# hustvl/ControlAR

Hardware: AMD Instinct MI355X
Metric: images/sec/GPU, LlamaGen-XL t2i canny 512x512 (1024 tok); 1/2/4/8-GPU scaling (higher is better)
Workload: dtype bf16

## Files before the change

controlar_amd/csrc/decode2.hip:

```cpp
#include "car_common.h"

typedef __attribute__((ext_vector_type(4))) unsigned u32x4;
typedef __attribute__((ext_vector_type(2))) float f32x2_t;
typedef __attribute__((ext_vector_type(2))) __bf16 bf16x2_t;

__device__ inline unsigned pack_bf16x2(float a, float b) {
    const f32x2_t v = {a, b};
    const bf16x2_t r = __builtin_convertvector(v, bf16x2_t);
    return *(const unsigned*)&r;
}

#include "decode2_params.h"

#ifdef CAR_STAMP
#define STAMP(p, i) do { if (threadIdx.x == 0 && (p).stamp) { const int wg_ = (int)(blockIdx.x + gridDim.x * (blockIdx.y + gridDim.y * blockIdx.z)); \
    if (wg_ < 2048) (p).stamp[((long)(p).stamp_slot * 2048 + wg_) * 8 + (i)] = (long long)wall_clock64(); } } while (0)
#else
#define STAMP(p, i) do { } while (0)
#endif

template <typename P>
__device__ inline void car_pf_helper_kv(const P& p, int hidx, unsigned& acc) {
    if (!p.pf_kc) return;
    const int x = (int)(blockIdx.x & 7), R = p.pf_wgs >> 3, r = hidx >> 3, nth = (int)blockDim.x, tid = (int)threadIdx.x;
    if (r >= R) return;
    const int pos = *p.pf_pos;
    const unsigned L = (unsigned)((((pos >> 5) + 1) * 32 * 64 * p.pf_kvb) >> 7);
    const unsigned nix = (unsigned)((p.pf_items - x + 7) >> 3);
    const unsigned tot = nix * 2u * L, step = (unsigned)(R * nth);
    const size_t stream = (size_t)p.pf_SA * 64 * p.pf_kvb;
    for (unsigned i = (unsigned)(r * nth + tid); i < tot; i += step) {
        const unsigned it = i / (2u * L), rem = i - it * 2u * L;
        const char* base = (const char*)(rem < L ? p.pf_kc : p.pf_vc) + (size_t)(x + 8 * (int)it) * stream;
        acc ^= *(const unsigned*)(base + (size_t)(rem < L ? rem : rem - L) * 128);
    }
}
__device__ inline void car_pf_helper(const void* p0, unsigned b0, const void* p1, unsigned b1, int hidx, int pf_wgs) {
    const int x = (int)(blockIdx.x & 7), R = pf_wgs >> 3, r = hidx >> 3, nth = (int)blockDim.x, tid = (int)threadIdx.x;
    if (r >= R) return;
    unsigned acc = 0;
#pragma unroll
    for (int job = 0; job < 2; ++job) {
        const unsigned* q = (const unsigned*)(job ? p1 : p0);
        const unsigned lines = (job ? b1 : b0) >> 7;
        if (!q || !lines) continue;
        const unsigned per = (lines + 7) >> 3, lo = (unsigned)x * per, hi = lo + per < lines ? lo + per : lines;
        const unsigned step = (unsigned)(R * nth);
        for (unsigned i = lo + (unsigned)(r * nth + tid); i < hi; i += step * 8) {
            unsigned v[8];
#pragma unroll
            for (int u = 0; u < 8; ++u) { const unsigned j = i + (unsigned)u * step; v[u] = 0; if (j < hi) v[u] = q[(size_t)j * 32]; }
#pragma unroll
            for (int u = 0; u < 8; ++u) acc ^= v[u];
        }
    }
    asm volatile("" ::"v"(acc));
}

typedef __attribute__((address_space(1))) const void car_gptr_t;
typedef __attribute__((address_space(3))) void car_lptr_t;

__device__ inline float sat448(float v) { return __builtin_amdgcn_fmed3f(v, -448.0f, 448.0f); }

__device__ inline bf16x8 fp8x8_to_bf16x8_(unsigned lo, unsigned hi) {
    const bf16x2_t a = __builtin_amdgcn_cvt_scalef32_pk_bf16_fp8(lo, 1.0f, false), b = __builtin_amdgcn_cvt_scalef32_pk_bf16_fp8(lo, 1.0f, true);
    const bf16x2_t c = __builtin_amdgcn_cvt_scalef32_pk_bf16_fp8(hi, 1.0f, false), d = __builtin_amdgcn_cvt_scalef32_pk_bf16_fp8(hi, 1.0f, true);
    u32x4 r;
    r[0] = *(const unsigned*)&a; r[1] = *(const unsigned*)&b; r[2] = *(const unsigned*)&c; r[3] = *(const unsigned*)&d;
    return *(bf16x8*)&r;
}

__device__ inline long bf16x8_to_fp8x8_(const u32x4 x) {
    int lo = 0, hi = 0;
#define CL(v) __builtin_amdgcn_fmed3f((v), -448.0f, 448.0f)
    lo = __builtin_amdgcn_cvt_pk_fp8_f32(CL(__uint_as_float(x[0] << 16)), CL(__uint_as_float(x[0] & 0xffff0000u)), lo, false);
    lo = __builtin_amdgcn_cvt_pk_fp8_f32(CL(__uint_as_float(x[1] << 16)), CL(__uint_as_float(x[1] & 0xffff0000u)), lo, true);
    hi = __builtin_amdgcn_cvt_pk_fp8_f32(CL(__uint_as_float(x[2] << 16)), CL(__uint_as_float(x[2] & 0xffff0000u)), hi, false);
    hi = __builtin_amdgcn_cvt_pk_fp8_f32(CL(__uint_as_float(x[3] << 16)), CL(__uint_as_float(x[3] & 0xffff0000u)), hi, true);
#undef CL
    return (long)(((unsigned long long)(unsigned)hi << 32) | (unsigned long long)(unsigned)lo);
}

template <int I, int J, int WAVES, int EPI, int F8, int NORM>
__global__ __launch_bounds__(WAVES * 64) void dec_gemm_kernel(GemmDP p) {
    extern __shared__ __attribute__((aligned(16))) float red_all[];
    static_assert((NORM != 1 && NORM != 3) || J == 1, "the prologue-norm and staged-norm variants serve one m-block");
    const int xs_ld = p.K + 8;
    bf16_t* xs = (bf16_t*)red_all;
    float* red = NORM == 1 ? red_all + (16 * xs_ld) / 2 : (NORM == 3 ? red_all + ((size_t)WAVES * p.stg) / 4 : red_all);
    constexpr int XPU = F8 ? 2 : 1;
    if (J == 1 && WAVES >= 8) car_kernarg_prefetch<(sizeof(GemmDP) + 63 + 48) / 64>();
    const int tid = threadIdx.x, lane = tid & 63, wave = tid >> 6;
    if (p.pf_wgs > 0 && (int)blockIdx.x >= (int)gridDim.x - p.pf_wgs) {
        STAMP(p, 0);
        car_pf_helper(p.pf_p0, p.pf_b0, p.pf_p1, p.pf_b1, (int)blockIdx.x - ((int)gridDim.x - p.pf_wgs), p.pf_wgs);
        { unsigned acc = 0; car_pf_helper_kv(p, (int)blockIdx.x - ((int)gridDim.x - p.pf_wgs), acc); asm volatile("" ::"v"(acc)); }
        STAMP(p, 5);
        return;
    }
    if (p.w_nt & 2) __builtin_amdgcn_s_setprio(3);
    STAMP(p, 0);
    const int nkb = p.K >> 5, nku = nkb / XPU, Mb = (p.M + 15) >> 4;
    const int MT = (Mb + J - 1) / J;
    int t = blockIdx.x; const int total = (int)gridDim.x - p.pf_wgs;
    if ((total & 7) == 0) t = (t & 7) * (total >> 3) + (t >> 3);
    const int nt = (NORM == 3) ? t : t / MT, mt = t - nt * MT;
    const int rb0 = nt * I, mb0 = mt * J;
    const int jn = (Mb - mb0) < J ? (Mb - mb0) : J;
    const int ku_lo = (int)((long)nku * wave / WAVES), ku_hi = (int)((long)nku * (wave + 1) / WAVES);
    const u32x4* wp = (const u32x4*)p.W + (long)rb0 * nku * 64 + lane;
    const u32x4* xp = (const u32x4*)p.X + (long)mb0 * nkb * 64 + lane;

    f32x4 acc[I][J];
#pragma unroll
    for (int i = 0; i < I; ++i)
#pragma unroll
        for (int j = 0; j < J; ++j) acc[i][j] = (f32x4){0.f, 0.f, 0.f, 0.f};
    const u32x4 zw = (u32x4){0u, 0u, 0u, 0u};
    constexpr int DEPTH = WAVES == 16 ? 8 : ((28 / (I + J * XPU)) < 2 ? 2 : ((28 / (I + J * XPU)) > 6 ? 6 : (28 / (I + J * XPU))));
    u32x4 wr[DEPTH][I], xr[DEPTH][J * XPU], nr[DEPTH][NORM == 2 ? XPU : 1];
    const bf16_t* hrow[J]; bool hok[J]; float rstd[J];
#pragma unroll
    for (int j = 0; j < J; ++j) { const int m = (mb0 + j) * 16 + (lane & 15); hok[j] = NORM == 2 && m < p.M; hrow[j] = NORM == 2 ? p.nh_in + (long)(hok[j] ? m : 0) * p.K + (lane >> 4) * 8 : nullptr; rstd[j] = 0.f; }
    auto loadW = [&](u32x4 (&w)[I], u32x4 (&nwf)[NORM == 2 ? XPU : 1], int ku) {
#pragma unroll
        for (int i = 0; i < I; ++i) {
            const u32x4* a = wp + ((long)i * nku + ku) * 64;
            w[i] = (p.w_nt & 1) ? __builtin_nontemporal_load(a) : *a;
        }
        if (NORM == 2) {
#pragma unroll
            for (int u = 0; u < XPU; ++u) nwf[u] = *(const u32x4*)(p.nw + (ku * XPU + u) * 32 + (lane >> 4) * 8);
        }
    };
    auto loadX = [&](u32x4 (&x)[J * XPU], int ku) {
        if (NORM == 0) {
#pragma unroll
            for (int j = 0; j < J; ++j)
#pragma unroll
                for (int u = 0; u < XPU; ++u) { x[j * XPU + u] = zw; if (j < jn) x[j * XPU + u] = xp[((long)j * nkb + ku * XPU + u) * 64]; }
        } else if (NORM == 2) {
#pragma unroll
            for (int j = 0; j < J; ++j)
#pragma unroll
                for (int u = 0; u < XPU; ++u) { x[j * XPU + u] = zw; if (hok[j]) x[j * XPU + u] = *(const u32x4*)(hrow[j] + (ku * XPU + u) * 32); }
        }
    };
    auto load = [&](u32x4 (&w)[I], u32x4 (&x)[J * XPU], u32x4 (&nwf)[NORM == 2 ? XPU : 1], int ku) { loadW(w, nwf, ku); loadX(x, ku); };
    const bf16_t* xl = xs + (lane & 15) * xs_ld + (lane >> 4) * 8;
    const int s_nkbw = NORM == 3 ? (ku_hi - ku_lo) * XPU : 0;
    const int s_xr = NORM == 3 ? (p.M * ((nku + WAVES - 1) / WAVES) * XPU * 4 + 63) >> 6 : 0;
    const int s_row = (lane & 15) < p.M ? (lane & 15) : p.M - 1;
    const char* stg_x = (const char*)red_all + (size_t)wave * (NORM == 3 ? p.stg : 0);
    const char* stg_w = stg_x + (size_t)s_xr * 1024;
    const char* stg_s = stg_w + 1024;
    auto compute = [&](const u32x4 (&w)[I], u32x4 (&x)[J * XPU], const u32x4 (&nwf)[NORM == 2 ? XPU : 1], int ku) {
        if (NORM == 1) {
#pragma unroll
            for (int u = 0; u < XPU; ++u) x[u] = *(const u32x4*)(xl + (ku * XPU + u) * 32);
        } else if (NORM == 3) {
#pragma unroll
            for (int u = 0; u < XPU; ++u) {
                const int kq = ((ku - ku_lo) * XPU + u) * 4 + (lane >> 4);
                x[u] = *(const u32x4*)(stg_x + ((size_t)s_row * (s_nkbw * 4) + kq) * 16);
                const u32x4 wq = *(const u32x4*)(stg_w + (size_t)kq * 16);
#pragma unroll
                for (int e = 0; e < 4; ++e) {
                    const unsigned hv = x[u][e], wv = wq[e];
                    const unsigned t = pack_bf16x2(__uint_as_float(hv << 16) * rstd[0], __uint_as_float(hv & 0xffff0000u) * rstd[0]);
                    x[u][e] = pack_bf16x2(__uint_as_float(t << 16) * __uint_as_float(wv << 16), __uint_as_float(t & 0xffff0000u) * __uint_as_float(wv & 0xffff0000u));
                }
            }
        } else if (NORM == 2) {
#pragma unroll
            for (int j = 0; j < J; ++j)
#pragma unroll
                for (int u = 0; u < XPU; ++u)
#pragma unroll
                    for (int e = 0; e < 4; ++e) {
                        const unsigned hv = x[j * XPU + u][e], wv = nwf[u][e];
                        const unsigned t = pack_bf16x2(__uint_as_float(hv << 16) * rstd[j], __uint_as_float(hv & 0xffff0000u) * rstd[j]);
                        x[j * XPU + u][e] = pack_bf16x2(__uint_as_float(t << 16) * __uint_as_float(wv << 16), __uint_as_float(t & 0xffff0000u) * __uint_as_float(wv & 0xffff0000u));
                    }
        }
        long x8[J][2];
        if (F8 == 2) {
#pragma unroll
            for (int j = 0; j < J; ++j) { x8[j][0] = bf16x8_to_fp8x8_(x[j * XPU]); x8[j][1] = bf16x8_to_fp8x8_(x[j * XPU + XPU - 1]); }
        }
#pragma unroll
        for (int i = 0; i < I; ++i) {
            if (F8 == 2) {
                const long a0 = (long)(((unsigned long long)w[i][1] << 32) | w[i][0]), a1 = (long)(((unsigned long long)w[i][3] << 32) | w[i][2]);
#pragma unroll
                for (int j = 0; j < J; ++j) {
                    acc[i][j] = __builtin_amdgcn_mfma_f32_16x16x32_fp8_fp8(a0, x8[j][0], acc[i][j], 0, 0, 0);
                    acc[i][j] = __builtin_amdgcn_mfma_f32_16x16x32_fp8_fp8(a1, x8[j][1], acc[i][j], 0, 0, 0);
                }
            } else if (F8) {
                const bf16x8 a0 = fp8x8_to_bf16x8_(w[i][0], w[i][1]), a1 = fp8x8_to_bf16x8_(w[i][2], w[i][3]);
#pragma unroll
                for (int j = 0; j < J; ++j) {
                    acc[i][j] = __builtin_amdgcn_mfma_f32_16x16x32_bf16(a0, *(const bf16x8*)&x[j * XPU], acc[i][j], 0, 0, 0);
                    acc[i][j] = __builtin_amdgcn_mfma_f32_16x16x32_bf16(a1, *(const bf16x8*)&x[j * XPU + XPU - 1], acc[i][j], 0, 0, 0);
                }
            } else {
#pragma unroll
                for (int j = 0; j < J; ++j)
                    acc[i][j] = __builtin_amdgcn_mfma_f32_16x16x32_bf16(*(const bf16x8*)&w[i], *(const bf16x8*)&x[j], acc[i][j], 0, 0, 0);
            }
        }
    };
    const int nkw = ku_hi - ku_lo;
    uint2 nh[8], na[8], nwv[8];
    bool n_add = false;
    if (NORM == 1) {
        const int D = p.K, ng = D >> 2;
        if (wave < p.M) {
            const int m = wave;
            const bf16_t* src = p.nidx ? p.nemb + (long)p.nidx[m] * D : p.nh_in + (long)m * D;
            const bf16_t* add = p.nadd ? p.nctrl + ((long)m * p.n_tok + (*p.pos - p.nT + 1)) * D : nullptr;
            n_add = add != nullptr;
#pragma unroll
            for (int q = 0; q < 8; ++q) {
                const int gi = lane + q * 64;
                if (gi < ng) { nh[q] = *(const uint2*)(src + gi * 4); nwv[q] = *(const uint2*)(p.nw + gi * 4); if (add) na[q] = *(const uint2*)(add + gi * 4); }
            }
        }
    }
    float4 sv[(NORM == 2 && J <= 2) ? J : 1][8];
    auto ssq_issue = [&](float4 (&v)[8], int j) {
        const int np4 = p.ssq_np >> 2, q4n = lane >> 4;
        const float4* sp = (const float4*)(p.ssq_in + (long)((mb0 + j) * 16 + (lane & 15)) * p.ssq_np);
#pragma unroll
        for (int t = 0; t < 8; ++t) { v[t] = make_float4(0.f, 0.f, 0.f, 0.f); if (hok[j] && q4n + 4 * t < np4) { const u32x4 r = *(const u32x4*)(sp + q4n + 4 * t); v[t] = make_float4(__uint_as_float(r[0]), __uint_as_float(r[1]), __uint_as_float(r[2]), __uint_as_float(r[3])); } }
    };
    auto ssq_finish = [&](const float4 (&v)[8], int j) {
        float sum = 0.f;
#pragma unroll
        for (int t = 0; t < 8; ++t) { sum += v[t].x; sum += v[t].y; sum += v[t].z; sum += v[t].w; }
        sum += __shfl_xor(sum, 16, 64); sum += __shfl_xor(sum, 32, 64);
        rstd[j] = hok[j] ? rsqrtf(sum / p.K + p.neps) : 0.f;
    };
    constexpr int IPc = I >= 2 ? I / 2 : 1, IWc = I >= 2 ? 2 : 1;
    const bool epi_first = wave < IPc * J && p.M <= 16;
    uint2 hv_h[IWc]; float4 cs_h[IWc];
    int pos_h = 0;
    if (EPI == EPI_QKV && p.M <= 16) pos_h = *(const __attribute__((address_space(4))) int*)(unsigned long long)p.pos;
    if (EPI == EPI_RESID && epi_first) {
        const int ip0 = wave / J, j0 = wave - ip0 * J;
        int m0 = (mb0 + j0) * 16 + (lane & 15); m0 = m0 < p.M ? m0 : p.M - 1;
#pragma unroll
        for (int ii = 0; ii < IWc; ++ii) hv_h[ii] = *(const uint2*)(p.h + (long)m0 * p.N + (rb0 + ip0 * IWc + ii) * 16 + (lane >> 4) * 4);
    }
    auto rope_first = [&]() {
        if (EPI == EPI_QKV && epi_first) {
            const int ip0 = wave / J;
#pragma unroll
            for (int ii = 0; ii < IWc; ++ii) {
                const int n0 = (rb0 + ip0 * IWc + ii) * 16 + (lane >> 4) * 4, d0 = (n0 % p.dim) & 63;
                cs_h[ii] = *(const float4*)(p.rope + ((long)pos_h * 32 + (d0 >> 1)) * 2);
            }
        }
    };
    if (NORM == 3 && s_nkbw > 0) {
        const int c4 = s_nkbw * 4, xtot = p.M * c4, kb0 = ku_lo * XPU;
        for (int r = 0; r < s_xr; ++r) {
            int ci = lane + 64 * r; ci = ci < xtot ? ci : xtot - 1;
            const int m = ci / c4, k8 = ci - m * c4;
            __builtin_amdgcn_global_load_lds((car_gptr_t*)(p.nh_in + (long)m * p.K + kb0 * 32 + k8 * 8), (car_lptr_t*)(stg_x + (size_t)r * 1024), 16, 0, 0);
        }
        { const int ci = lane < c4 ? lane : c4 - 1;
          __builtin_amdgcn_global_load_lds((car_gptr_t*)(p.nw + kb0 * 32 + ci * 8), (car_lptr_t*)stg_w, 16, 0, 0); }
        const int stot = p.M * (p.ssq_np >> 2), sr = (stot + 63) >> 6;
        for (int r = 0; r < sr; ++r) {
            int ci = lane + 64 * r; ci = ci < stot ? ci : stot - 1;
            __builtin_amdgcn_global_load_lds((car_gptr_t*)(p.ssq_in + (long)ci * 4), (car_lptr_t*)(stg_s + (size_t)r * 1024), 16, 0, 0);
        }
    }
    if (NORM == 2) {
#pragma unroll
        for (int j = 0; j < J; ++j) { if (J <= 2) ssq_issue(sv[j], j); else { ssq_issue(sv[0], j); ssq_finish(sv[0], j); } }
    }
#pragma unroll
    for (int d = 0; d < DEPTH; ++d) if (d < nkw) load(wr[d], xr[d], nr[d], ku_lo + d);
    rope_first();
    STAMP(p, 6);
    if (NORM == 3) {
        asm volatile("s_waitcnt vmcnt(0)" ::: "memory");
        const int np4 = p.ssq_np >> 2, q4n = lane >> 4;
        float sum = 0.f;
        for (int t = 0; 4 * t < np4; ++t) {
            const int ci = q4n + 4 * t;
            const float4 v = *(const float4*)(stg_s + ((size_t)s_row * np4 + (ci < np4 ? ci : np4 - 1)) * 16);
            const bool ok = ci < np4;
            sum += ok ? v.x : 0.f; sum += ok ? v.y : 0.f; sum += ok ? v.z : 0.f; sum += ok ? v.w : 0.f;
        }
        sum += __shfl_xor(sum, 16, 64); sum += __shfl_xor(sum, 32, 64);
        rstd[0] = (lane & 15) < p.M ? rsqrtf(sum / p.K + p.neps) : 0.f;
    }
    if (NORM == 2 && J <= 2) {
#pragma unroll
        for (int j = 0; j < J; ++j) ssq_finish(sv[J <= 2 ? j : 0], j);
    }
    if (NORM == 1) {
        const int D = p.K, ng = D >> 2;
        for (int m = wave; m < p.M; m += WAVES) {
            if (m != wave) {
                const bf16_t* src = p.nidx ? p.nemb + (long)p.nidx[m] * D : p.nh_in + (long)m * D;
                const bf16_t* add = p.nadd ? p.nctrl + ((long)m * p.n_tok + (*p.pos - p.nT + 1)) * D : nullptr;
                n_add = add != nullptr;
#pragma unroll
                for (int q = 0; q < 8; ++q) {
                    const int gi = lane + q * 64;
                    if (gi < ng) { nh[q] = *(const uint2*)(src + gi * 4); if (add) na[q] = *(const uint2*)(add + gi * 4); }
                }
            }
            float val[8][4];
            float ss = 0.f;
#pragma unroll
            for (int q = 0; q < 8; ++q) {
                const int gi = lane + q * 64;
                if (gi < ng) {
                    const uint2 u = nh[q];
                    float v[4] = {__uint_as_float(u.x << 16), __uint_as_float(u.x & 0xffff0000u), __uint_as_float(u.y << 16), __uint_as_float(u.y & 0xffff0000u)};
                    if (n_add) {
                        const uint2 a = na[q];
                        const float c[4] = {__uint_as_float(a.x << 16), __uint_as_float(a.x & 0xffff0000u), __uint_as_float(a.y << 16), __uint_as_float(a.y & 0xffff0000u)};
#pragma unroll
                        for (int e = 0; e < 4; ++e) v[e] = bf2f(f2bf(v[e] + bf2f(f2bf(p.ncs * c[e]))));
                    }
#pragma unroll
                    for (int e = 0; e < 4; ++e) { val[q][e] = v[e]; ss += v[e] * v[e]; }
                }
            }
            const float rstd = rsqrtf(wave_sum(ss) / D + p.neps);
#pragma unroll
            for (int q = 0; q < 8; ++q) {
                const int gi = lane + q * 64;
                if (gi < ng) {
                    const int k = gi * 4;
                    if (p.nh_out && blockIdx.x == 0) { uint2 u; u.x = pack_bf16x2(val[q][0], val[q][1]); u.y = pack_bf16x2(val[q][2], val[q][3]); *(uint2*)(p.nh_out + (long)m * D + k) = u; }
                    const uint2 wu = nwv[q];
                    const float w[4] = {__uint_as_float(wu.x << 16), __uint_as_float(wu.x & 0xffff0000u), __uint_as_float(wu.y << 16), __uint_as_float(wu.y & 0xffff0000u)};
                    uint2 u;
                    u.x = pack_bf16x2(bf2f(f2bf(val[q][0] * rstd)) * w[0], bf2f(f2bf(val[q][1] * rstd)) * w[1]);
                    u.y = pack_bf16x2(bf2f(f2bf(val[q][2] * rstd)) * w[2], bf2f(f2bf(val[q][3] * rstd)) * w[3]);
                    *(uint2*)(xs + m * xs_ld + k) = u;
                }
            }
        }
        __syncthreads();
    }
    STAMP(p, 1);
    for (int base = 0; base < nkw; base += DEPTH) {
#pragma unroll
        for (int d = 0; d < DEPTH; ++d) {
            if (base + d < nkw) {
                compute(wr[d], xr[d], nr[d], ku_lo + base + d);
#ifdef CAR_STAMP
                if (base + d == 0) { asm volatile("s_nop 0" ::"v"(acc[0][0][0])); STAMP(p, 2); }
#endif
                if (base + d + DEPTH < nkw) load(wr[d], xr[d], nr[d], ku_lo + base + d + DEPTH);
            }
        }
    }
    f32x4* rv = (f32x4*)red;
#ifdef CAR_STAMP
    asm volatile("s_nop 0" ::"v"(acc[0][0][0])); STAMP(p, 3);
#endif
#pragma unroll
    for (int i = 0; i < I; ++i)
#pragma unroll
        for (int j = 0; j < J; ++j) rv[((wave * I + i) * J + j) * 64 + lane] = acc[i][j];
    __syncthreads();
    STAMP(p, 4);
    auto fold = [&](int i, int j) -> f32x4 {
        f32x4 s = rv[((0 * I + i) * J + j) * 64 + lane];
        for (int w = 1; w < WAVES; ++w) { const f32x4 v = rv[((w * I + i) * J + j) * 64 + lane]; s[0] += v[0]; s[1] += v[1]; s[2] += v[2]; s[3] += v[3]; }
        return s;
    };
    constexpr int IP = I >= 2 ? I / 2 : 1, IW = I >= 2 ? 2 : 1;
    const int q4 = lane >> 4, c16 = lane & 15;
    for (int u = wave; u < IP * J; u += WAVES) {
        const bool first_u = u == wave && epi_first;
        const int ip = u / J, j = u - ip * J;
        if (j >= jn) continue;
        const int m = (mb0 + j) * 16 + c16;
        f32x4 v[IW];
#pragma unroll
        for (int ii = 0; ii < IW; ++ii) {
            v[ii] = fold(ip * IW + ii, j);
            if (F8) {
                const float4 sc = *(const float4*)(p.wscale + (rb0 + ip * IW + ii) * 16 + q4 * 4);
                v[ii][0] *= sc.x; v[ii][1] *= sc.y; v[ii][2] *= sc.z; v[ii][3] *= sc.w;
            }
        }
        if (m >= p.M) continue;
        if (EPI == EPI_SWIGLU) {
            float s[4];
#pragma unroll
            for (int r = 0; r < 4; ++r) {
                const float a = bf2f(f2bf(v[0][r])), g = bf2f(f2bf(v[IW - 1][r]));
                s[r] = bf2f(f2bf(silu_f(a))) * g;
            }
            const int hid = ((rb0 >> 1) + ip) * 16 + q4 * 4;
            const int nkb2 = p.N >> 6;
            const long off = ((((long)(m >> 4) * nkb2 + (hid >> 5)) * 64 + ((hid & 31) >> 3) * 16 + (m & 15)) << 3) + (hid & 7);
            uint2 o; o.x = pack_bf16x2(s[0], s[1]); o.y = pack_bf16x2(s[2], s[3]);
            *(uint2*)(p.outp + off) = o;
        } else {
            float ssq_acc = 0.f;
#pragma unroll
            for (int ii = 0; ii < IW; ++ii) {
                const int n0 = (rb0 + ip * IW + ii) * 16 + q4 * 4;
                const f32x4 a = v[ii];
                if (EPI == EPI_LOGITS) {
                    float4 o; o.x = bf2f(f2bf(a[0])); o.y = bf2f(f2bf(a[1])); o.z = bf2f(f2bf(a[2])); o.w = bf2f(f2bf(a[3]));
                    *(float4*)(p.outf + (long)m * p.N + n0) = o;
                } else if (EPI == EPI_RESID) {
                    bf16_t* hp = p.h + (long)m * p.N + n0;
                    const uint2 hv = first_u ? hv_h[ii] : *(const uint2*)hp;
                    const float h0 = __uint_as_float(hv.x << 16), h1 = __uint_as_float(hv.x & 0xffff0000u);
                    const float h2 = __uint_as_float(hv.y << 16), h3 = __uint_as_float(hv.y & 0xffff0000u);
                    uint2 o;
                    o.x = pack_bf16x2(h0 + bf2f(f2bf(a[0])), h1 + bf2f(f2bf(a[1])));
                    o.y = pack_bf16x2(h2 + bf2f(f2bf(a[2])), h3 + bf2f(f2bf(a[3])));
                    *(uint2*)hp = o;
                    if (p.ssq_out) {
                        const float s0 = __uint_as_float(o.x << 16), s1 = __uint_as_float(o.x & 0xffff0000u), s2 = __uint_as_float(o.y << 16), s3 = __uint_as_float(o.y & 0xffff0000u);
                        ssq_acc += s0 * s0; ssq_acc += s1 * s1; ssq_acc += s2 * s2; ssq_acc += s3 * s3;
                    }
                } else {
                    const int pos = p.M <= 16 ? pos_h : *p.pos;
                    const int sec = n0 / p.dim, within = n0 - sec * p.dim, hh = within >> 6, d0 = within & 63;
                    const float x0 = bf2f(f2bf(a[0])), x1 = bf2f(f2bf(a[1])), x2 = bf2f(f2bf(a[2])), x3 = bf2f(f2bf(a[3]));
                    const long sb = ((long)m * p.H + hh) * p.SA * 64;
                    if (sec == 2) {
                        const int w = pos & 31, qv = w < 16 ? (w >> 2) : ((w - 16) >> 2), ev = w < 16 ? (w & 3) : (4 + ((w - 16) & 3));
                        if (p.kv8) {
                            unsigned char* vb = (unsigned char*)p.vc + sb + (long)(pos >> 5) * 2048 + (d0 >> 5) * 1024 + ((qv * 16 + (d0 & 15)) << 4) + ((d0 >> 4) & 1) * 8 + ev;
                            const int e01 = __builtin_amdgcn_cvt_pk_fp8_f32(sat448(x0), sat448(x1), 0, false), e23 = __builtin_amdgcn_cvt_pk_fp8_f32(sat448(x2), sat448(x3), 0, false);
                            vb[0] = (unsigned char)(e01 & 0xff); vb[16] = (unsigned char)((e01 >> 8) & 0xff); vb[32] = (unsigned char)(e23 & 0xff); vb[48] = (unsigned char)((e23 >> 8) & 0xff);
                        } else {
                            bf16_t* vb = p.vc + sb + ((long)(pos >> 5) * 4 + (d0 >> 4)) * 512 + ((qv * 16 + (d0 & 15)) << 3) + ev;
                            vb[0] = f2bf(x0); vb[8] = f2bf(x1); vb[16] = f2bf(x2); vb[24] = f2bf(x3);
                        }
                    } else {
                        const float4 cs = first_u ? cs_h[ii] : *(const float4*)(p.rope + ((long)pos * 32 + (d0 >> 1)) * 2);
                        const float r0 = x0 * cs.x - x1 * cs.y, r1 = x1 * cs.x + x0 * cs.y;
                        const float r2 = x2 * cs.z - x3 * cs.w, r3 = x3 * cs.z + x2 * cs.w;
                        if (sec == 0) {
                            uint2 o;
                            o.x = pack_bf16x2(bf2f(f2bf(r0)) * 0.125f, bf2f(f2bf(r1)) * 0.125f);
                            o.y = pack_bf16x2(bf2f(f2bf(r2)) * 0.125f, bf2f(f2bf(r3)) * 0.125f);
                            *(uint2*)(p.qout + ((long)m * p.H + hh) * 64 + d0) = o;
                        } else if (p.kv8) {
                            unsigned char* kb_ = (unsigned char*)p.kc + sb + (long)(pos >> 4) * 1024 + ((((d0 & 31) >> 3) * 16 + (pos & 15)) << 4) + (d0 >> 5) * 8 + (d0 & 7);
                            int e = __builtin_amdgcn_cvt_pk_fp8_f32(sat448(bf2f(f2bf(r0))), sat448(bf2f(f2bf(r1))), 0, false);
                            e = __builtin_amdgcn_cvt_pk_fp8_f32(sat448(bf2f(f2bf(r2))), sat448(bf2f(f2bf(r3))), e, true);
                            *(unsigned*)kb_ = (unsigned)e;
                        } else {
                            uint2 o; o.x = pack_bf16x2(r0, r1); o.y = pack_bf16x2(r2, r3);
                            bf16_t* kb_ = p.kc + sb + ((long)(pos >> 4) * 2 + (d0 >> 5)) * 512 + ((((d0 & 31) >> 3) * 16 + (pos & 15)) << 3) + (d0 & 7);
                            *(uint2*)kb_ = o;
                        }
                    }
                }
            }
            if (EPI == EPI_RESID && p.ssq_out) {
                ssq_acc += __shfl_xor(ssq_acc, 16, 64); ssq_acc += __shfl_xor(ssq_acc, 32, 64);
                if (q4 == 0) *(unsigned*)(p.ssq_out + (long)m * p.ssq_ld + (rb0 / IW + ip)) = __float_as_uint(ssq_acc);
            }
        }
    }
#ifdef CAR_STAMP
    __builtin_amdgcn_s_waitcnt(0); STAMP(p, 5);
#endif
}

template <int I, int J, int WAVES, int F8, int NORM>
static void launch_gemm_ij(const GemmDP& p_, int epi, hipStream_t st) {
    GemmDP p = p_;
    const int Mb = (p.M + 15) / 16, MT = (Mb + J - 1) / J, NT = p.N / (16 * I);
    const dim3 g(NT * MT + (p.pf_wgs > 0 ? p.pf_wgs : 0)), b(WAVES * 64);
    if (NORM == 3) {
        const int nku = p.K / (F8 ? 64 : 32), xr = (p.M * ((nku + WAVES - 1) / WAVES) * (F8 ? 2 : 1) * 4 + 63) / 64, sr = (p.M * (p.ssq_np / 4) + 63) / 64;
        p.stg = (xr + 1 + sr) * 1024;
    }
    const size_t sh = (size_t)WAVES * I * J * 64 * 16 + (NORM == 1 ? (size_t)16 * (p.K + 8) * 2 : 0) + (NORM == 3 ? (size_t)WAVES * p.stg : 0);
    static size_t attr[4] = {0, 0, 0, 0};
#define LG(E)                                                                                                                   \
    do {                                                                                                                        \
        if (sh > 48 * 1024 && sh > attr[E]) { (void)hipFuncSetAttribute((const void*)dec_gemm_kernel<I, J, WAVES, E, F8, NORM>, hipFuncAttributeMaxDynamicSharedMemorySize, (int)sh); attr[E] = sh; } \
        hipLaunchKernelGGL((dec_gemm_kernel<I, J, WAVES, E, F8, NORM>), g, b, sh, st, p);                                        \
    } while (0)
    if (NORM) {
        if (epi == EPI_LOGITS) LG(EPI_LOGITS); else if (epi == EPI_SWIGLU) LG(EPI_SWIGLU); else LG(EPI_QKV);
    } else {
        if (epi == EPI_LOGITS) LG(EPI_LOGITS); else if (epi == EPI_RESID) LG(EPI_RESID); else if (epi == EPI_SWIGLU) LG(EPI_SWIGLU); else LG(EPI_QKV);
    }
#undef LG
}

extern "C" int car_launch_dec_gemm_cfg_ex(const GemmDP* p, int epi, int cfg, int staged_ok, hipStream_t st) {
    if (epi == EPI_SWIGLU && cfg < 200) return -1;
    if (p->N % (16 * (cfg / 100)) || p->K % 32) return -1;
    if (p->wscale && p->K % 64) return -1;
    const int f8 = p->wscale ? (p->f8_mfma ? 2 : 1) : 0;
    if (p->ssq_in) {
        if (!p->nw || !p->nh_in || epi == EPI_RESID || p->ssq_np <= 0 || (p->ssq_np & 3) || p->ssq_np > 128) return -1;
        {
            const int nku = p->K / (f8 ? 64 : 32), nkw_max = (nku + 7) / 8;
            if (p->M <= 16 && (cfg / 10) % 10 == 1 && cfg % 10 == 1 && nku >= 8 && nkw_max * (f8 ? 2 : 1) <= 16 && staged_ok) {
                switch (cfg / 100) {
#define CASE3(I) case I: if (f8 == 2) launch_gemm_ij<I, 1, 8, 2, 3>(*p, epi, st); else if (f8) launch_gemm_ij<I, 1, 8, 1, 3>(*p, epi, st); else launch_gemm_ij<I, 1, 8, 0, 3>(*p, epi, st); return 0;
                    CASE3(1) CASE3(2) CASE3(4)
#undef CASE3
                    default: break;
                }
            }
        }
        switch (cfg) {
#define CASE(I, J) case I * 100 + J * 10: if (f8 == 2) launch_gemm_ij<I, J, 4, 2, 2>(*p, epi, st); else if (f8) launch_gemm_ij<I, J, 4, 1, 2>(*p, epi, st); else launch_gemm_ij<I, J, 4, 0, 2>(*p, epi, st); break; \
                   case I * 100 + J * 10 + 1: if (f8 == 2) launch_gemm_ij<I, J, 8, 2, 2>(*p, epi, st); else if (f8) launch_gemm_ij<I, J, 8, 1, 2>(*p, epi, st); else launch_gemm_ij<I, J, 8, 0, 2>(*p, epi, st); break;
            CASE(1, 1) CASE(1, 2) CASE(1, 4) CASE(2, 1) CASE(2, 2) CASE(2, 4) CASE(4, 1) CASE(4, 2) CASE(4, 4)
#undef CASE
            default: return -1;
        }
        return 0;
    }
    if (p->nw) {
        if (p->M > 16 || (cfg / 10) % 10 != 1 || epi == EPI_RESID || p->K > 2048) return -1;
        switch (cfg) {
#define CASE(I) case I * 100 + 10: if (f8 == 2) launch_gemm_ij<I, 1, 4, 2, 1>(*p, epi, st); else if (f8) launch_gemm_ij<I, 1, 4, 1, 1>(*p, epi, st); else launch_gemm_ij<I, 1, 4, 0, 1>(*p, epi, st); break; \
                case I * 100 + 11: if (f8 == 2) launch_gemm_ij<I, 1, 8, 2, 1>(*p, epi, st); else if (f8) launch_gemm_ij<I, 1, 8, 1, 1>(*p, epi, st); else launch_gemm_ij<I, 1, 8, 0, 1>(*p, epi, st); break;
            CASE(1) CASE(2) CASE(4)
#undef CASE
            default: return -1;
        }
        return 0;
    }
    switch (cfg) {
#define CASE(I, J) case I * 100 + J * 10: if (f8 == 2) launch_gemm_ij<I, J, 4, 2, 0>(*p, epi, st); else if (f8) launch_gemm_ij<I, J, 4, 1, 0>(*p, epi, st); else launch_gemm_ij<I, J, 4, 0, 0>(*p, epi, st); break; \
                   case I * 100 + J * 10 + 1: if (f8 == 2) launch_gemm_ij<I, J, 8, 2, 0>(*p, epi, st); else if (f8) launch_gemm_ij<I, J, 8, 1, 0>(*p, epi, st); else launch_gemm_ij<I, J, 8, 0, 0>(*p, epi, st); break;
        CASE(1, 1) CASE(1, 2) CASE(1, 4) CASE(2, 1) CASE(2, 2) CASE(2, 4) CASE(4, 1) CASE(4, 2) CASE(4, 4)
#undef CASE
        case 112: if (f8 == 2) launch_gemm_ij<1, 1, 16, 2, 0>(*p, epi, st); else if (f8) launch_gemm_ij<1, 1, 16, 1, 0>(*p, epi, st); else launch_gemm_ij<1, 1, 16, 0, 0>(*p, epi, st); break;
        default: return -1;
    }
    return 0;
}

extern "C" int car_launch_dec_gemm_cfg(const GemmDP* p, int epi, int cfg, hipStream_t st) { return car_launch_dec_gemm_cfg_ex(p, epi, cfg, 1, st); }
extern "C" int car_pick_gemm_cfg(int M, int N, int K, int epi) {
    const int Mb = (M + 15) / 16;
    const bool wideN = N >= 6144, hugeN = N >= 16384, longK = K >= 2048, smallNK = N <= 1536 && K <= 1536;
    int cfg;
    if (Mb >= 12) cfg = wideN ? 440 : 241;
    else if (Mb >= 6) cfg = hugeN ? 440 : (wideN ? 441 : (smallNK ? 110 : 221));
    else if (Mb >= 3) cfg = hugeN ? 441 : (wideN ? 241 : (longK ? 211 : 110));
    else if (Mb == 2) cfg = hugeN ? 421 : (wideN ? 221 : (longK ? 121 : 120));
    else cfg = hugeN ? 411 : (wideN ? 211 : 111);
    if (Mb == 1 && epi == EPI_RESID && cfg == 111 && N / 16 <= 128) cfg = 112;
    int I = cfg / 100;
    if (epi == EPI_SWIGLU && I < 2) I = 2;
    while (I > 1 && N % (16 * I)) I >>= 1;
    return I * 100 + cfg % 100;
}

extern "C" void car_launch_dec_gemm(const GemmDP* p, int epi, hipStream_t st) {
    (void)car_launch_dec_gemm_cfg(p, epi, car_pick_gemm_cfg(p->M, p->N, p->K, epi), st);
}

template <int NWAVE, int PF, int KV8>
__global__ __launch_bounds__(NWAVE * 64) void dec_attn2_kernel(Attn2P p) {
    __shared__ float red[NWAVE][66];
    const int split = blockIdx.z;
    const int tid = threadIdx.x, lane = tid & 63, wave = tid >> 6, q4 = lane >> 4, c16 = lane & 15;
    STAMP(p, 0);
    const int pos = *p.pos;
    const bool persist = p.n_seq > 0;
    const int n_items = persist ? p.n_seq * p.H : 1;
    for (int it = persist ? (int)blockIdx.x : 0; it < n_items; it += gridDim.x) {
    const int h = persist ? it % p.H : (int)blockIdx.x, b = persist ? it / p.H : (int)blockIdx.y;
    const long sbase = ((long)b * p.H + h) * p.SA * 64;
    const u32x4* Kp = KV8 ? (const u32x4*)((const unsigned char*)p.kc + sbase) + lane : (const u32x4*)(p.kc + sbase) + lane;
    const u32x4* Vp = KV8 ? (const u32x4*)((const unsigned char*)p.vc + sbase) + lane : (const u32x4*)(p.vc + sbase) + lane;
    const bf16_t* qp = p.q + ((long)b * p.H + h) * 64;
    const bf16x8 qf0 = *(const bf16x8*)(qp + q4 * 8), qf1 = *(const bf16x8*)(qp + 32 + q4 * 8);
    const unsigned char* mk = p.mask ? p.mask + (long)b * p.T : nullptr;
    int jmin = 0;
    if (mk) {
        if (p.jmin) jmin = p.jmin[b];
        else {
            int jm = p.T;
            for (int j = lane; j < p.T; j += 64) { const int v = mk[j]; if (v != 0 && j < jm) jm = j; }
#pragma unroll
            for (int o = 32; o > 0; o >>= 1) jm = min(jm, __shfl_xor(jm, o, 64));
            jmin = jm;
        }
    }
    const int nblk = (pos >> 5) + 1, NW = p.nsplit * NWAVE;
    float m_run = -INFINITY, l_run = 0.f;
    f32x4 o[4];
#pragma unroll
    for (int d = 0; d < 4; ++d) o[d] = (f32x4){0.f, 0.f, 0.f, 0.f};
    const f32x4 z4 = (f32x4){0.f, 0.f, 0.f, 0.f};

    auto load = [&](u32x4 (&kr)[4], u32x4 (&vr)[4], unsigned (&mb)[8], int blk) {
        if (mk != nullptr && blk * 32 < p.T) {
            const int jb = blk * 32 + q4 * 4;
#pragma unroll
            for (int e = 0; e < 8; ++e) mb[e] = mk[min(jb + (e < 4 ? e : 12 + e), p.T - 1)];
        }
#pragma unroll
        for (int i = 0; i < (KV8 ? 2 : 4); ++i) kr[i] = __builtin_nontemporal_load(Kp + ((long)blk * (KV8 ? 2 : 4) + i) * 64);
#pragma unroll
        for (int i = 0; i < (KV8 ? 2 : 4); ++i) vr[i] = __builtin_nontemporal_load(Vp + ((long)blk * (KV8 ? 2 : 4) + i) * 64);
    };
    auto compute = [&](const u32x4 (&kr_)[4], const u32x4 (&vr_)[4], const unsigned (&mb)[8], int blk) {
        u32x4 kr[4], vr[4];
        if (KV8) {
#pragma unroll
            for (int i = 0; i < 2; ++i) {
                const bf16x8 a = fp8x8_to_bf16x8_(kr_[i][0], kr_[i][1]), c2 = fp8x8_to_bf16x8_(kr_[i][2], kr_[i][3]);
                const bf16x8 v0 = fp8x8_to_bf16x8_(vr_[i][0], vr_[i][1]), v1 = fp8x8_to_bf16x8_(vr_[i][2], vr_[i][3]);
                kr[2 * i] = *(const u32x4*)&a; kr[2 * i + 1] = *(const u32x4*)&c2; vr[2 * i] = *(const u32x4*)&v0; vr[2 * i + 1] = *(const u32x4*)&v1;
            }
        } else {
#pragma unroll
            for (int i = 0; i < 4; ++i) { kr[i] = kr_[i]; vr[i] = vr_[i]; }
        }
        f32x4 s0 = __builtin_amdgcn_mfma_f32_16x16x32_bf16(*(const bf16x8*)&kr[0], qf0, z4, 0, 0, 0);
        s0 = __builtin_amdgcn_mfma_f32_16x16x32_bf16(*(const bf16x8*)&kr[1], qf1, s0, 0, 0, 0);
        f32x4 s1 = __builtin_amdgcn_mfma_f32_16x16x32_bf16(*(const bf16x8*)&kr[2], qf0, z4, 0, 0, 0);
        s1 = __builtin_amdgcn_mfma_f32_16x16x32_bf16(*(const bf16x8*)&kr[3], qf1, s1, 0, 0, 0);
        float sc[8] = {s0[0], s0[1], s0[2], s0[3], s1[0], s1[1], s1[2], s1[3]};
        const int jb = blk * 32 + q4 * 4;
        const bool use_mk = mk != nullptr && blk * 32 < p.T;
        if (use_mk || blk * 32 + 31 > pos) {
#pragma unroll
            for (int e = 0; e < 8; ++e) {
                const int j = jb + (e < 4 ? e : 12 + e);
                unsigned mv = 1u;
                if (use_mk) mv = mb[e];
                const bool ok = (j <= pos) & ((j >= p.T) | (mv != 0u));
                sc[e] = ok ? sc[e] : -INFINITY;
            }
        }
        float mx = fmaxf(fmaxf(fmaxf(sc[0], sc[1]), fmaxf(sc[2], sc[3])), fmaxf(fmaxf(sc[4], sc[5]), fmaxf(sc[6], sc[7])));
        mx = fmaxf(mx, __shfl_xor(mx, 16, 64)); mx = fmaxf(mx, __shfl_xor(mx, 32, 64));
        if (mx > -INFINITY) {
            const float mn = fmaxf(m_run, mx), alpha = __expf(m_run - mn);
            float pe[8], ps = 0.f;
#pragma unroll
            for (int e = 0; e < 8; ++e) { pe[e] = __expf(sc[e] - mn); ps += pe[e]; }
            l_run = l_run * alpha + ps; m_run = mn;
            u32x4 pu; pu[0] = pack_bf16x2(pe[0], pe[1]); pu[1] = pack_bf16x2(pe[2], pe[3]); pu[2] = pack_bf16x2(pe[4], pe[5]); pu[3] = pack_bf16x2(pe[6], pe[7]);
#pragma unroll
            for (int d = 0; d < 4; ++d) {
                o[d][0] *= alpha; o[d][1] *= alpha; o[d][2] *= alpha; o[d][3] *= alpha;
                o[d] = __builtin_amdgcn_mfma_f32_16x16x32_bf16(*(const bf16x8*)&pu, *(const bf16x8*)&vr[d], o[d], 0, 0, 0);
            }
        }
    };
    if (PF) {
        u32x4 ka[4], va[4], kb2[4], vb2[4]; unsigned ma[8], mb2[8];
        int blk = (jmin >> 5) + split * NWAVE + wave;
        if (blk < nblk) load(ka, va, ma, blk);
        while (blk < nblk) {
            int nb = blk + NW;
            if (nb < nblk) load(kb2, vb2, mb2, nb);
            compute(ka, va, ma, blk);
            blk = nb;
            if (blk >= nblk) break;
            nb = blk + NW;
            if (nb < nblk) load(ka, va, ma, nb);
            compute(kb2, vb2, mb2, blk);
            blk = nb;
        }
    } else {
        u32x4 ka[4], va[4]; unsigned ma[8];
        for (int blk = (jmin >> 5) + split * NWAVE + wave; blk < nblk; blk += NW) { load(ka, va, ma, blk); compute(ka, va, ma, blk); }
    }
#ifdef CAR_STAMP
    asm volatile("s_nop 0" ::"v"(l_run)); STAMP(p, 3);
#endif
    float lt = l_run + __shfl_xor(l_run, 16, 64); lt += __shfl_xor(lt, 32, 64);
    if (q4 == 0) {
#pragma unroll
        for (int d = 0; d < 4; ++d) red[wave][2 + d * 16 + c16] = o[d][0];
    }
    if (lane == 0) { red[wave][0] = m_run; red[wave][1] = lt; }
    __syncthreads();
    STAMP(p, 4);
    if (tid < 64) {
        float M = red[0][0];
#pragma unroll
        for (int w = 1; w < NWAVE; ++w) M = fmaxf(M, red[w][0]);
        float L = 0.f, O = 0.f;
#pragma unroll
        for (int w = 0; w < NWAVE; ++w) {
            const float mm = red[w][0];
            const float a = mm > -INFINITY ? __expf(mm - M) : 0.f;
            L += red[w][1] * a; O += red[w][2 + tid] * a;
        }
        if (p.nsplit == 1) {
            const int k = h * 64 + tid;
            long off;
            if (p.out_packed) off = ((((long)(b >> 4) * (p.dim >> 5) + (k >> 5)) * 64 + ((k & 31) >> 3) * 16 + (b & 15)) << 3) + (k & 7);
            else off = (long)b * p.dim + k;
            p.out[off] = f2bf(O / L);
        } else {
            float* pt = p.part + (((long)b * p.H + h) * p.nsplit + split) * 66;
            if (tid == 0) { pt[0] = M; pt[1] = L; }
            pt[2 + tid] = O;
        }
    }
    if (persist) __syncthreads();
    }
    if (persist && p.pf_wgs > 0 && (int)blockIdx.x >= n_items) car_pf_helper(p.pf_p0, p.pf_b0, p.pf_p1, p.pf_b1, (int)blockIdx.x - n_items, p.pf_wgs);
#ifdef CAR_STAMP
    __builtin_amdgcn_s_waitcnt(0); STAMP(p, 5);
#endif
}

template <int KV8>
__global__ __launch_bounds__(1024) void dec_attn2s_kernel(Attn2P p) {
    __shared__ float red[16][66];
    car_kernarg_prefetch<(sizeof(Attn2P) + 63 + 48) / 64>();
    const int tid = threadIdx.x, lane = tid & 63, wave = tid >> 6, q4 = lane >> 4, c16 = lane & 15;
    STAMP(p, 0);
    const int n_items = p.n_seq * p.H;
    if ((int)blockIdx.x >= n_items) {
        car_pf_helper(p.pf_p0, p.pf_b0, p.pf_p1, p.pf_b1, (int)blockIdx.x - n_items, p.pf_wgs);
#ifdef CAR_STAMP
        __builtin_amdgcn_s_waitcnt(0); STAMP(p, 5);
#endif
        return;
    }
    const int h = (int)blockIdx.x % p.H, b = (int)blockIdx.x / p.H;
    const int pos = *p.pos;
    const unsigned char* mk = p.mask ? p.mask + (long)b * p.T : nullptr;
    const int jmin = mk ? p.jmin[b] : 0;
    const long sbase = ((long)b * p.H + h) * p.SA * 64;
    const u32x4* Kp = KV8 ? (const u32x4*)((const unsigned char*)p.kc + sbase) + lane : (const u32x4*)(p.kc + sbase) + lane;
    const u32x4* Vp = KV8 ? (const u32x4*)((const unsigned char*)p.vc + sbase) + lane : (const u32x4*)(p.vc + sbase) + lane;
    const bf16_t* qp = p.q + ((long)b * p.H + h) * 64;
    bf16x8 qf0, qf1;
    const int nblk = (pos >> 5) + 1;
    float m_run = -INFINITY, l_run = 0.f;
    f32x4 o[4];
#pragma unroll
    for (int d = 0; d < 4; ++d) o[d] = (f32x4){0.f, 0.f, 0.f, 0.f};
    const f32x4 z4 = (f32x4){0.f, 0.f, 0.f, 0.f};
    constexpr int NL = KV8 ? 2 : 4;
    auto loadkv = [&](u32x4 (&kr)[4], u32x4 (&vr)[4], int blk) {
#pragma unroll
        for (int i = 0; i < NL; ++i) kr[i] = __builtin_nontemporal_load(Kp + ((long)blk * NL + i) * 64);
#pragma unroll
        for (int i = 0; i < NL; ++i) vr[i] = __builtin_nontemporal_load(Vp + ((long)blk * NL + i) * 64);
    };
    unsigned ma[8];
    auto compute = [&](const u32x4 (&kr_)[4], const u32x4 (&vr_)[4], int blk, bool use_mk) {
        u32x4 kr[4], vr[4];
        if (KV8) {
#pragma unroll
            for (int i = 0; i < 2; ++i) {
                const bf16x8 a = fp8x8_to_bf16x8_(kr_[i][0], kr_[i][1]), c2 = fp8x8_to_bf16x8_(kr_[i][2], kr_[i][3]);
                const bf16x8 v0 = fp8x8_to_bf16x8_(vr_[i][0], vr_[i][1]), v1 = fp8x8_to_bf16x8_(vr_[i][2], vr_[i][3]);
                kr[2 * i] = *(const u32x4*)&a; kr[2 * i + 1] = *(const u32x4*)&c2; vr[2 * i] = *(const u32x4*)&v0; vr[2 * i + 1] = *(const u32x4*)&v1;
            }
        } else {
#pragma unroll
            for (int i = 0; i < 4; ++i) { kr[i] = kr_[i]; vr[i] = vr_[i]; }
        }
        f32x4 s0 = __builtin_amdgcn_mfma_f32_16x16x32_bf16(*(const bf16x8*)&kr[0], qf0, z4, 0, 0, 0);
        s0 = __builtin_amdgcn_mfma_f32_16x16x32_bf16(*(const bf16x8*)&kr[1], qf1, s0, 0, 0, 0);
        f32x4 s1 = __builtin_amdgcn_mfma_f32_16x16x32_bf16(*(const bf16x8*)&kr[2], qf0, z4, 0, 0, 0);
        s1 = __builtin_amdgcn_mfma_f32_16x16x32_bf16(*(const bf16x8*)&kr[3], qf1, s1, 0, 0, 0);
        float sc[8] = {s0[0], s0[1], s0[2], s0[3], s1[0], s1[1], s1[2], s1[3]};
        const int jb = blk * 32 + q4 * 4;
        if (use_mk || blk * 32 + 31 > pos) {
#pragma unroll
            for (int e = 0; e < 8; ++e) {
                const int j = jb + (e < 4 ? e : 12 + e);
                unsigned mv = 1u;
                if (use_mk) mv = ma[e];
                const bool ok = (j <= pos) & ((j >= p.T) | (mv != 0u));
                sc[e] = ok ? sc[e] : -INFINITY;
            }
        }
        float mx = fmaxf(fmaxf(fmaxf(sc[0], sc[1]), fmaxf(sc[2], sc[3])), fmaxf(fmaxf(sc[4], sc[5]), fmaxf(sc[6], sc[7])));
        mx = fmaxf(mx, __shfl_xor(mx, 16, 64)); mx = fmaxf(mx, __shfl_xor(mx, 32, 64));
        if (mx > -INFINITY) {
            const float mn = fmaxf(m_run, mx), alpha = __expf(m_run - mn);
            float pe[8], ps = 0.f;
#pragma unroll
            for (int e = 0; e < 8; ++e) { pe[e] = __expf(sc[e] - mn); ps += pe[e]; }
            l_run = l_run * alpha + ps; m_run = mn;
            u32x4 pu; pu[0] = pack_bf16x2(pe[0], pe[1]); pu[1] = pack_bf16x2(pe[2], pe[3]); pu[2] = pack_bf16x2(pe[4], pe[5]); pu[3] = pack_bf16x2(pe[6], pe[7]);
#pragma unroll
            for (int d = 0; d < 4; ++d) {
                o[d][0] *= alpha; o[d][1] *= alpha; o[d][2] *= alpha; o[d][3] *= alpha;
                o[d] = __builtin_amdgcn_mfma_f32_16x16x32_bf16(*(const bf16x8*)&pu, *(const bf16x8*)&vr[d], o[d], 0, 0, 0);
            }
        }
    };
    {
        u32x4 ka[4], va[4], kb2[4], vb2[4];
        int cur = (jmin >> 5) + wave;
        const bool mk_a = mk != nullptr && cur * 32 < p.T && cur < nblk;
        if (mk_a) {
            const int jb = cur * 32 + q4 * 4;
#pragma unroll
            for (int e = 0; e < 8; ++e) ma[e] = mk[min(jb + (e < 4 ? e : 12 + e), p.T - 1)];
        }
        if (cur < nblk) loadkv(ka, va, cur);
        if (cur + 16 < nblk) loadkv(kb2, vb2, cur + 16);
        { const u32x4 q0 = *(const u32x4*)(qp + q4 * 8), q1 = *(const u32x4*)(qp + 32 + q4 * 8); qf0 = *(const bf16x8*)&q0; qf1 = *(const bf16x8*)&q1; }
        bool first = true;
        while (cur < nblk) {
            compute(ka, va, cur, first && mk_a);
            first = false;
            if (cur + 32 < nblk) loadkv(ka, va, cur + 32);
            if (cur + 16 < nblk) { compute(kb2, vb2, cur + 16, false); if (cur + 48 < nblk) loadkv(kb2, vb2, cur + 48); }
            cur += 32;
        }
    }
#ifdef CAR_STAMP
    asm volatile("s_nop 0" ::"v"(l_run)); STAMP(p, 3);
#endif
    float lt = l_run + __shfl_xor(l_run, 16, 64); lt += __shfl_xor(lt, 32, 64);
    if (q4 == 0) {
#pragma unroll
        for (int d = 0; d < 4; ++d) red[wave][2 + d * 16 + c16] = o[d][0];
    }
    if (lane == 0) { red[wave][0] = m_run; red[wave][1] = lt; }
    __syncthreads();
    STAMP(p, 4);
    if (tid < 64) {
        float M = red[0][0];
#pragma unroll
        for (int w = 1; w < 16; ++w) M = fmaxf(M, red[w][0]);
        float L = 0.f, O = 0.f;
#pragma unroll
        for (int w = 0; w < 16; ++w) {
            const float mm = red[w][0];
            const float a = mm > -INFINITY ? __expf(mm - M) : 0.f;
            L += red[w][1] * a; O += red[w][2 + tid] * a;
        }
        const int k = h * 64 + tid;
        long off;
        if (p.out_packed) off = ((((long)(b >> 4) * (p.dim >> 5) + (k >> 5)) * 64 + ((k & 31) >> 3) * 16 + (b & 15)) << 3) + (k & 7);
        else off = (long)b * p.dim + k;
        p.out[off] = f2bf(O / L);
    }
#ifdef CAR_STAMP
    __builtin_amdgcn_s_waitcnt(0); STAMP(p, 5);
#endif
}

__global__ void build_mask_kernel(const int64_t* emb_mask, const int* row_img, unsigned char* out, int b, int T) {
    const long i = (long)blockIdx.x * blockDim.x + threadIdx.x;
    if (i >= (long)b * T) return;
    const int r = (int)(i / T), t = (int)(i - (long)r * T);
    out[i] = emb_mask ? (unsigned char)(emb_mask[(long)row_img[r] * T + t] != 0) : (unsigned char)1;
}
extern "C" void car_launch_build_mask(const int64_t* emb_mask, const int* row_img, unsigned char* out, int b, int T, hipStream_t st) {
    const long n = (long)b * T;
    hipLaunchKernelGGL(build_mask_kernel, dim3((unsigned)((n + 255) / 256)), dim3(256), 0, st, emb_mask, row_img, out, b, T);
}

__global__ void mask_first_valid_kernel(const unsigned char* mask, int* jmin, int T) {
    const int b = blockIdx.x, lane = threadIdx.x;
    int jm = T;
    for (int j = lane; j < T; j += 64) { const int v = mask[(long)b * T + j]; if (v != 0 && j < jm) jm = j; }
#pragma unroll
    for (int o = 32; o > 0; o >>= 1) jm = min(jm, __shfl_xor(jm, o, 64));
    if (lane == 0) jmin[b] = jm;
}
extern "C" void car_launch_mask_first_valid(const unsigned char* mask, int* jmin, int b, int T, hipStream_t st) {
    hipLaunchKernelGGL(mask_first_valid_kernel, dim3(b), dim3(64), 0, st, mask, jmin, T);
}
__global__ __launch_bounds__(256) void min_int_kernel(const int* v, int n, int* out, int need, int* flag) {
    __shared__ int sm[4];
    int m = 0x7fffffff;
    for (int i = threadIdx.x; i < n; i += 256) m = min(m, v[i]);
#pragma unroll
    for (int o = 32; o > 0; o >>= 1) m = min(m, __shfl_xor(m, o, 64));
    if ((threadIdx.x & 63) == 0) sm[threadIdx.x >> 6] = m;
    __syncthreads();
    if (threadIdx.x == 0) { const int r = min(min(sm[0], sm[1]), min(sm[2], sm[3])); out[0] = r; if (flag && need >= 0 && r < need) *flag = 1; }
}
extern "C" void car_launch_min_int(const int* v, int n, int* out, int need, int* flag, hipStream_t st) { hipLaunchKernelGGL(min_int_kernel, dim3(1), dim3(256), 0, st, v, n, out, need, flag); }

__global__ __launch_bounds__(64) void dec_attn2_combine_kernel(const float* part, bf16_t* out, int H, int nsplit, int dim, int out_packed) {
    const int h = blockIdx.x, b = blockIdx.y, d = threadIdx.x;
    const float* pt = part + ((long)b * H + h) * nsplit * 66;
    float M = -INFINITY;
    for (int s = 0; s < nsplit; ++s) M = fmaxf(M, pt[s * 66]);
    float L = 0.f, O = 0.f;
    for (int s = 0; s < nsplit; ++s) {
        const float mm = pt[s * 66];
        if (mm > -INFINITY) { const float a = __expf(mm - M); L += pt[s * 66 + 1] * a; O += pt[s * 66 + 2 + d] * a; }
    }
    const int k = h * 64 + d;
    long off;
    if (out_packed) off = ((((long)(b >> 4) * (dim >> 5) + (k >> 5)) * 64 + ((k & 31) >> 3) * 16 + (b & 15)) << 3) + (k & 7);
    else off = (long)b * dim + k;
    out[off] = f2bf(O / L);
}

extern "C" void car_launch_dec_attn2_var(const Attn2P* p, int b, int variant, int lds_pad, hipStream_t st) {
    if (variant == 162 && p->nsplit == 1 && p->T <= 512 && (!p->mask || p->jmin)) {
        Attn2P q = *p; q.n_seq = b; q.pgrid = 0;
        if (q.pf_wgs < 0 || ((b * q.H) & 7)) q.pf_wgs = 0;
        const dim3 g(b * q.H + q.pf_wgs);
        if (q.kv8) hipLaunchKernelGGL((dec_attn2s_kernel<1>), g, dim3(1024), 0, st, q); else hipLaunchKernelGGL((dec_attn2s_kernel<0>), g, dim3(1024), 0, st, q);
        return;
    }
    if (variant == 162) variant = 160;
    const bool persist = p->n_seq > 0 && p->pgrid > 0 && p->nsplit == 1;
    Attn2P q = *p; if (!persist) { q.n_seq = 0; q.pgrid = 0; q.pf_wgs = 0; }
    p = &q;
    const dim3 g = persist ? dim3(q.pgrid, 1, 1) : dim3(p->H, b, p->nsplit);
    const size_t sh = (size_t)(lds_pad > 0 ? lds_pad : 0);
#define LA(NW, PF_) do { if (p->kv8) hipLaunchKernelGGL((dec_attn2_kernel<NW, PF_, 1>), g, dim3(NW * 64), sh, st, *p); else hipLaunchKernelGGL((dec_attn2_kernel<NW, PF_, 0>), g, dim3(NW * 64), sh, st, *p); } while (0)
    switch (variant) {
        case 20: LA(2, 0); break;
        case 21: LA(2, 1); break;
        case 40: LA(4, 0); break;
        case 80: LA(8, 0); break;
        case 81: LA(8, 1); break;
        case 160: LA(16, 0); break;
        case 161: LA(16, 1); break;
        default: LA(4, 1); break;
    }
#undef LA
    if (p->nsplit > 1 && p->out)
        hipLaunchKernelGGL(dec_attn2_combine_kernel, dim3(p->H, b), dim3(64), 0, st, p->part, p->out, p->H, p->nsplit, p->dim, p->out_packed);
}
extern "C" void car_launch_dec_attn2(const Attn2P* p, int b, hipStream_t st) { car_launch_dec_attn2_var(p, b, 40, 0, st); }
__global__ void prefill_rope_kv2_kernel(bf16_t* qkv, bf16_t* kcache, bf16_t* vcache, const float* rope, int b, int Tn, int H, int dim, int SA, int kv8, int t0) {
    const long total = (long)b * Tn * H * 32;
    long i = (long)blockIdx.x * blockDim.x + threadIdx.x;
    const long stride = (long)gridDim.x * blockDim.x;
    for (; i < total; i += stride) {
        const int pr = (int)(i % 32); const int h = (int)((i / 32) % H); const int tw = (int)((i / (32L * H)) % Tn); const long bb = i / (32L * H * Tn);
        bf16_t* row = qkv + (bb * Tn + tw) * 3 * dim;
        const int t = tw + t0;
        const float cs = rope[((long)t * 32 + pr) * 2], sn = rope[((long)t * 32 + pr) * 2 + 1];
        const float q0 = bf2f(row[h * 64 + 2 * pr]), q1 = bf2f(row[h * 64 + 2 * pr + 1]);
        const float k0 = bf2f(row[dim + h * 64 + 2 * pr]), k1 = bf2f(row[dim + h * 64 + 2 * pr + 1]);
        row[h * 64 + 2 * pr] = f2bf(q0 * cs - q1 * sn); row[h * 64 + 2 * pr + 1] = f2bf(q1 * cs + q0 * sn);
        const bf16_t kr0 = f2bf(k0 * cs - k1 * sn), kr1 = f2bf(k1 * cs + k0 * sn);
        row[dim + h * 64 + 2 * pr] = kr0; row[dim + h * 64 + 2 * pr + 1] = kr1;
        const long sb = (bb * H + h) * (long)SA * 64;
        const int d = 2 * pr;
        const int w = t & 31, qv = w < 16 ? (w >> 2) : ((w - 16) >> 2), ev = w < 16 ? (w & 3) : (4 + ((w - 16) & 3));
        if (kv8) {
            const int ek = __builtin_amdgcn_cvt_pk_fp8_f32(sat448(bf2f(kr0)), sat448(bf2f(kr1)), 0, false);
            unsigned char* kp = (unsigned char*)kcache + sb + (long)(t >> 4) * 1024 + ((((d & 31) >> 3) * 16 + (t & 15)) << 4) + (d >> 5) * 8 + (d & 7);
            kp[0] = (unsigned char)(ek & 0xff); kp[1] = (unsigned char)((ek >> 8) & 0xff);
            const int ev2 = __builtin_amdgcn_cvt_pk_fp8_f32(sat448(bf2f(row[2 * dim + h * 64 + d])), sat448(bf2f(row[2 * dim + h * 64 + d + 1])), 0, false);
            unsigned char* vp = (unsigned char*)vcache + sb + (long)(t >> 5) * 2048 + (d >> 5) * 1024 + ((qv * 16 + (d & 15)) << 4) + ((d >> 4) & 1) * 8 + ev;
            vp[0] = (unsigned char)(ev2 & 0xff); vp[16] = (unsigned char)((ev2 >> 8) & 0xff);
        } else {
            bf16_t* kp = kcache + sb + ((long)(t >> 4) * 2 + (d >> 5)) * 512 + ((((d & 31) >> 3) * 16 + (t & 15)) << 3) + (d & 7);
            kp[0] = kr0; kp[1] = kr1;
            bf16_t* vp = vcache + sb + ((long)(t >> 5) * 4 + (d >> 4)) * 512 + ((qv * 16 + (d & 15)) << 3) + ev;
            vp[0] = row[2 * dim + h * 64 + d]; vp[8] = row[2 * dim + h * 64 + d + 1];
        }
    }
}
extern "C" void car_launch_prefill_rope_kv2(void* qkv, void* kc, void* vc, const float* rope, int b, int Tn, int H, int dim, int SA, int kv8, int t0, hipStream_t st) {
    long total = (long)b * Tn * H * 32; int g = (int)((total + 255) / 256); if (g > 4096) g = 4096;
    hipLaunchKernelGGL(prefill_rope_kv2_kernel, dim3(g), dim3(256), 0, st, (bf16_t*)qkv, (bf16_t*)kc, (bf16_t*)vc, rope, b, Tn, H, dim, SA, kv8, t0);
}

template <int NQ>
__global__ __launch_bounds__(256) void rmsnorm2_kernel(Norm2P p, int rows) {
    car_kernarg_prefetch<(sizeof(Norm2P) + 63 + 48) / 64>();
    if (p.pf_wgs > 0 && (int)blockIdx.x >= (int)gridDim.x - p.pf_wgs) {
        STAMP(p, 0);
        car_pf_helper(p.pf_p0, p.pf_b0, p.pf_p1, p.pf_b1, (int)blockIdx.x - ((int)gridDim.x - p.pf_wgs), p.pf_wgs);
        STAMP(p, 5);
        return;
    }
    const long r = (long)blockIdx.x * 4 + (threadIdx.x >> 6);
    STAMP(p, 0);
    if (r < rows) {
    const int lane = threadIdx.x & 63;
    const int D = p.D, ng = D >> 2;
    const bf16_t* src = p.idx ? p.emb + (long)p.idx[r] * D : p.h_in + r * D;
    if (p.add & 2) __builtin_amdgcn_s_setprio(3);
    const bf16_t* add = (p.add & 1) ? p.ctrl + (r * p.n_tok + (*p.pos - p.T + 1)) * D : nullptr;
    float val[NQ][4];
    float ss = 0.f;
    uint2 wreg[NQ];
#pragma unroll
    for (int q = 0; q < NQ; ++q) { const int gi = lane + q * 64; if (gi < ng) wreg[q] = *(const uint2*)(p.w + gi * 4); }
#pragma unroll
    for (int q = 0; q < NQ; ++q) {
        const int gi = lane + q * 64;
        if (gi < ng) {
            const uint2 u = *(const uint2*)(src + gi * 4);
            float v[4] = {__uint_as_float(u.x << 16), __uint_as_float(u.x & 0xffff0000u), __uint_as_float(u.y << 16), __uint_as_float(u.y & 0xffff0000u)};
            if (add) {
                const uint2 a = *(const uint2*)(add + gi * 4);
                const float c[4] = {__uint_as_float(a.x << 16), __uint_as_float(a.x & 0xffff0000u), __uint_as_float(a.y << 16), __uint_as_float(a.y & 0xffff0000u)};
#pragma unroll
                for (int e = 0; e < 4; ++e) v[e] = bf2f(f2bf(v[e] + bf2f(f2bf(p.cs * c[e]))));
            }
#pragma unroll
            for (int e = 0; e < 4; ++e) { val[q][e] = v[e]; ss += v[e] * v[e]; }
        }
    }
    const float rstd = rsqrtf(wave_sum(ss) / D + p.eps);
#ifdef CAR_STAMP
    asm volatile("s_nop 0" ::"v"(rstd)); STAMP(p, 3);
#endif
    const int nkb = D >> 5;
#pragma unroll
    for (int q = 0; q < NQ; ++q) {
        const int gi = lane + q * 64;
        if (gi < ng) {
            const int k = gi * 4;
            if (p.h_out) { uint2 u; u.x = pack_bf16x2(val[q][0], val[q][1]); u.y = pack_bf16x2(val[q][2], val[q][3]); *(uint2*)(p.h_out + r * D + k) = u; }
            const uint2 wu = wreg[q];
            const float w[4] = {__uint_as_float(wu.x << 16), __uint_as_float(wu.x & 0xffff0000u), __uint_as_float(wu.y << 16), __uint_as_float(wu.y & 0xffff0000u)};
            float o[4];
#pragma unroll
            for (int e = 0; e < 4; ++e) o[e] = bf2f(f2bf(val[q][e] * rstd)) * w[e];
            uint2 u; u.x = pack_bf16x2(o[0], o[1]); u.y = pack_bf16x2(o[2], o[3]);
            const long off = ((((r >> 4) * nkb + (k >> 5)) * 64 + ((k & 31) >> 3) * 16 + (r & 15)) << 3) + (k & 7);
            *(uint2*)(p.xn + off) = u;
        }
    }
    }
#ifdef CAR_STAMP
    __builtin_amdgcn_s_waitcnt(0); STAMP(p, 5);
#endif
}
extern "C" void car_launch_rmsnorm2(const Norm2P* p, long rows, hipStream_t st) {
    const int nq = (p->D / 4 + 63) / 64;
    Norm2P q = *p;
    const unsigned main_wgs = (unsigned)((rows + 3) / 4);
    if (q.pf_wgs < 0 || (main_wgs & 7)) q.pf_wgs = 0;
    const dim3 g(main_wgs + (unsigned)q.pf_wgs), b(256);
    if (nq <= 4) hipLaunchKernelGGL((rmsnorm2_kernel<4>), g, b, 0, st, q, (int)rows);
    else if (nq <= 8) hipLaunchKernelGGL((rmsnorm2_kernel<8>), g, b, 0, st, q, (int)rows);
    else hipLaunchKernelGGL((rmsnorm2_kernel<16>), g, b, 0, st, q, (int)rows);
}
```

controlar_amd/csrc/decode2_params.h:

```cpp
#pragma once
#include "car_common.h"

#define CAR_GEMMDP_DEFINED
#ifdef CAR_STAMP
#define CAR_STAMP_FIELDS long long* stamp; int stamp_slot;
#else
#define CAR_STAMP_FIELDS
#endif
enum { EPI_LOGITS = 0, EPI_RESID = 1, EPI_SWIGLU = 2, EPI_QKV = 3 };

#define CAR_PF_FIELDS const void* pf_p0; const void* pf_p1; unsigned pf_b0, pf_b1; int pf_wgs; const void* pf_kc; const void* pf_vc; const int* pf_pos; int pf_items, pf_SA, pf_kvb;

struct GemmDP {
    const bf16_t* W;
    const bf16_t* X;
    int M, N, K;
    int w_nt;
    int f8_mfma;
    const float* wscale;
    bf16_t* h;
    bf16_t* outp;
    float* outf;
    bf16_t* qout;
    bf16_t* kc; bf16_t* vc;
    const float* rope;
    const int* pos;
    int H, SA, dim;
    int kv8;
    const bf16_t* nh_in; const bf16_t* nemb; const int* nidx; bf16_t* nh_out; const bf16_t* nw; const bf16_t* nctrl;
    int nadd, nT, n_tok; float ncs, neps;
    const float* ssq_in; int ssq_np;
    int stg;
    float* ssq_out; int ssq_ld;
    CAR_PF_FIELDS
    CAR_STAMP_FIELDS
};

struct Attn2P {
    const bf16_t* q;
    const bf16_t* kc; const bf16_t* vc;
    const int* pos;
    const unsigned char* mask;
    const int* jmin;
    bf16_t* out;
    float* part;
    int H, SA, T, dim, nsplit, out_packed;
    int kv8;
    int n_seq, pgrid;
    CAR_PF_FIELDS
    CAR_STAMP_FIELDS
};

struct Norm2P {
    const bf16_t* h_in; const bf16_t* emb; const int* idx; bf16_t* h_out; bf16_t* xn; const bf16_t* w;
    const bf16_t* ctrl; const int* pos; int add ; int T; int n_tok; float cs;
    int D; float eps;
    CAR_PF_FIELDS
    CAR_STAMP_FIELDS
};
```

controlar_amd/csrc/engine_generate.hip:

```cpp
#include "engine_internal.h"

enum { RA_NONE = 0, RA_SMALL, RA_NX, RA_MID, kEarlyChain = 8, kNoOverride = -0x7fffffff };
struct ChainPlan {
    int b0, bg, nsplit;
    int attn_variant, attn_lds_pad, attn_pgrid;
    int fuse_norm, normx, normx_max, normx_j4, staged_normx;
    int runahead, kv_runahead;
};
struct DecodePlan {
    int mode, NG, mult, img0[9];
    int phase, gsteps, lin_prio, no_graph;
    int n_early;
    int f32_resid_cfg, f32_qkv_tiled_from;
    ChainPlan ch[9];
};
static int attn_splits(int wg) { int n = 1; while (wg * n < 1024 && n < 16) n *= 2; return n; }

static void plan_decode(DecodePlan& pl, const car_config& g, int mode, int n_cu, int B, bool use_cfg, int S_max, int nsteps, int skip, bool has_mask) {
    memset(&pl, 0, sizeof(pl));
    const bool fast = mode == CAR_BF16;
    const int D = g.dim, Hn = g.n_head, Fh = g.ffn_hidden, V = g.vocab_size, T = g.cls_token_num;
    const int mult = use_cfg ? 2 : 1, b = mult * B;
    auto num = [](const char* v, int dflt) { return v ? atoi(v) : dflt; };
    const char *k_chains = CAR_KNOB("CAR_CHAINS"), *k_one_max = CAR_KNOB("CAR_ONE_LAUNCH_MAX"), *k_variant = CAR_KNOB("CAR_ATTN_VARIANT"), *k_phase = CAR_KNOB("CAR_PHASE_OFFSET"), *k_form = CAR_KNOB("CAR_ATTN_F32_FORM");
    const bool single_chain = CAR_KNOB("CAR_SINGLE_CHAIN"), no_early = CAR_KNOB("CAR_NO_EARLY_CHAIN"), split_small = CAR_KNOB("CAR_ATTN_SPLIT_SMALL"), old_small = CAR_KNOB("CAR_ATTN_OLD_SMALL");
    const bool no_runahead = CAR_KNOB("CAR_NO_RUNAHEAD"), no_small_fuse = CAR_KNOB("CAR_NO_SMALL_FUSE"), no_normx = CAR_KNOB("CAR_NO_NORMX"), kv_runahead = CAR_KNOB("CAR_KV_RUNAHEAD"), no_staged = CAR_KNOB("CAR_NO_STAGED_NORMX");
    const int k_nsplit = num(CAR_KNOB("CAR_ATTN_NSPLIT"), 0), k_persist = num(CAR_KNOB("CAR_ATTN_PERSIST"), 0), lds_pad = num(CAR_KNOB("CAR_ATTN_LDS_PAD"), 0);
    const int normx_max = num(CAR_KNOB("CAR_NORMX_MAX"), 48), normx_j4 = num(CAR_KNOB("CAR_NORMX_J4"), 0) != 0, k_gsteps = num(CAR_KNOB("CAR_GRAPH_STEPS"), 1);
    pl.mode = mode; pl.mult = mult; pl.lin_prio = num(CAR_KNOB("CAR_LINEAR_PRIO"), 0) != 0;
    pl.no_graph = CAR_KNOB("CAR_NO_GRAPH") != nullptr;
    pl.f32_resid_cfg = num(CAR_KNOB("CAR_F32_RESID_CFG"), kNoOverride); pl.f32_qkv_tiled_from = num(CAR_KNOB("CAR_F32_QKV_TILED_FROM"), kNoOverride);

    int NG = b >= 192 ? 2 : 1;
    if (!fast && b >= 288) NG = 3;
    if (k_chains) { const int v = atoi(k_chains); if (v >= 1 && v <= 8 && B / v >= 2) NG = v; }
    if (single_chain || NG > B) NG = 1;
    pl.NG = NG; for (int gi = 0; gi <= NG; ++gi) pl.img0[gi] = (int)((long)B * gi / NG);
    pl.phase = NG >= 2 && (k_phase ? atoi(k_phase) != 0 : !fast);
    pl.gsteps = fast && k_gsteps >= 1 && k_gsteps <= 64 ? k_gsteps : 1;
    const int nsplit_exact = (S_max + AF_SPLIT - 1) / AF_SPLIT;
    const bool fused = (long)Hn * b >= 2048 && nsplit_exact <= 8;
    auto plan_exact = [&](ChainPlan& cp) { cp.nsplit = nsplit_exact; cp.attn_variant = fused ? num(k_form, cp.bg < b ? 3 : 1) : 0; };
    for (int gi = 0; gi < NG; ++gi) {
        ChainPlan& cp = pl.ch[gi]; const int bg = mult * (pl.img0[gi + 1] - pl.img0[gi]);
        cp.b0 = mult * pl.img0[gi]; cp.bg = bg;
        if (!fast) { plan_exact(cp); continue; }
        const bool one_launch = (long)bg * Hn <= num(k_one_max, T <= 512 ? 480 : 240) && !split_small;
        cp.nsplit = one_launch ? 1 : attn_splits(bg * Hn);
        if (k_nsplit == 1 || k_nsplit == 2 || k_nsplit == 4 || k_nsplit == 8 || k_nsplit == 16) cp.nsplit = k_nsplit;
        cp.attn_variant = (one_launch && cp.nsplit == 1) ? ((T <= 512 && !old_small) ? 162 : 160) : ((cp.nsplit == 1 && bg < 128) ? 20 : 40);
        cp.attn_variant = num(k_variant, cp.attn_variant); cp.attn_lds_pad = lds_pad;
        if (k_persist > 0 && k_persist <= 16 && cp.nsplit == 1) { const long items = (long)bg * Hn, cap = (long)n_cu * k_persist;
            if (items > cap) { const long per = (items + cap - 1) / cap; cp.attn_pgrid = (int)((items + per - 1) / per); }
        }
        cp.fuse_norm = bg <= 8 && D <= 2048 && !no_small_fuse;
        cp.normx_max = normx_max; cp.normx_j4 = normx_j4; cp.staged_normx = !no_staged;
        cp.normx = bg <= normx_max && D % 128 == 0 && D <= 2048 && !no_normx;
        if (n_cu >= 128 && !no_runahead) cp.runahead = bg <= 16 ? RA_SMALL : (bg != b ? RA_NONE : (bg <= normx_max ? RA_NX : RA_MID));
        cp.kv_runahead = kv_runahead && cp.attn_variant == 162 && ((bg * Hn) & 7) == 0;
    }
    if (!fast && NG == 3 && mult == 1 && !k_chains && !no_early) {
        const double P = (double)g.n_layer * (4.0 * D * D + 3.0 * (double)D * Fh) + (double)V * D;
        const int rows_star = (int)(0.087 * P / (8.0 * D * g.n_layer));
        const int attended0 = has_mask ? 24 : T;
        pl.n_early = std::min(rows_star - attended0 - skip, nsteps); if (pl.n_early < 8) pl.n_early = 0;
        pl.ch[kEarlyChain].bg = b; plan_exact(pl.ch[kEarlyChain]);
    }
}

struct FastBufs { bf16_t *xn, *att, *mid, *q; float* logits; float* attn_part; float* ssq; };
struct ChainBind { int *pos, *step; FastBufs fb; SampleP sp; };
struct StepBufs {
    void *h, *xn, *qkv, *att, *mid; float* part; float* logits; int* cur;
    int b, SA, n_tok; bool use_ctrl; float cs; const unsigned char* maskb; const int* jmin;
    ChainBind ch[9];
};

static int enqueue_decode_step_fast(car_ctx* c, const StepBufs& sb, const DecodePlan& pl, int ci, hipStream_t st, hipEvent_t phase_ev, hipStream_t phase_dst) {
    const car_config& g = c->cfg;
    const ChainPlan& cp = pl.ch[ci]; const ChainBind& cb = sb.ch[ci]; const FastBufs& fb = cb.fb;
    const int D = g.dim, Hn = g.n_head, Fh = g.ffn_hidden, li = g.n_layer / 3, V = g.vocab_size, T = g.cls_token_num;
    const int b = cp.bg, b0 = cp.b0, nsplit = cp.nsplit, SA = sb.SA, n_tok = sb.n_tok, prio = pl.lin_prio;
    const size_t kv_layer = (size_t)sb.b * Hn * SA * 64, kv_off = (size_t)b0 * Hn * SA * 64;
    bf16_t* h = (bf16_t*)sb.h + (size_t)b0 * D;
    const bool f8 = g.decode_weight_fp8 != 0;
    int nk = 0, bad_cfg = 0;
    const bool ra_lin = cp.runahead == RA_SMALL || cp.runahead == RA_NX, ra_norm = cp.runahead == RA_NX || cp.runahead == RA_MID;
    auto wimg = [&](const std::string& wname, const void*& ptr, unsigned& bytes, size_t cap = (size_t)24 << 20) {
        auto it = c->w.find(wname + (f8 ? "#pk8" : "#pk"));
        if (it == c->w.end()) { ptr = nullptr; bytes = 0; return; }
        ptr = it->second.p; bytes = (unsigned)std::min(it->second.bytes, cap);
    };
    auto helpers_for = [&](bool on, int main_wgs) -> int {
        if (!on || (main_wgs & 7)) return 0;
        const int n = std::min(((c->n_cu - main_wgs) / 8) * 8, 192);
        return n >= 32 ? n : 0;
    };
    auto ctrl_at = [&](int l) { return sb.use_ctrl && l < g.n_layer && l % li == 0 && l / li < 3; };
    auto gemm = [&](const std::string& wname, const bf16_t* X, int N, int K, int epi, GemmDP gp_) -> int {
        GemmDP p = gp_;
        p.W = (const bf16_t*)Wp(c, wname + (f8 ? "#pk8" : "#pk")); p.X = X; p.M = b; p.N = N; p.K = K;
        p.wscale = f8 ? (const float*)Wp(c, wname + "#sc") : nullptr; p.f8_mfma = g.decode_weight_fp8 == 2;
        int cfg = car_pick_gemm_cfg(b, N, K, epi);
        if (p.ssq_in && b > 48 && b <= 64 && cp.normx_j4) cfg = ((epi == EPI_SWIGLU || N >= 6144) ? 200 : 100) + 40 + 1;
        const int I = cfg / 100, J = (cfg / 10) % 10, Mb = (b + 15) / 16;
        p.w_nt = ((Mb + J - 1) / J == 1 ? 1 : 0) | (prio ? 2 : 0);
        if (p.pf_wgs > 0) p.pf_wgs = std::min(helpers_for(ra_lin, (N / (16 * I)) * ((Mb + J - 1) / J)), 160);
        if (p.ssq_out) p.ssq_ld = N / (16 * (I >= 2 ? 2 : 1));
        if (car_launch_dec_gemm_cfg_ex(&p, epi, cfg, cp.staged_normx, st)) bad_cfg = cfg;
        ++nk;
        return p.ssq_out ? p.ssq_ld : 0;
    };
    GemmDP z; memset(&z, 0, sizeof(z));
    int ssq_np = 0;
    bf16_t* hc = h;
    bf16_t* halt = (bf16_t*)sb.xn + (size_t)b0 * D;
    auto norm_kernel = [&](const std::string& wname, int l, const std::string& pf0, const std::string& pf1, size_t cap0 = (size_t)24 << 20) {
        Norm2P np; memset(&np, 0, sizeof(np));
        np.h_in = h; np.xn = fb.xn; np.w = (const bf16_t*)Wp(c, wname); np.D = D; np.eps = g.norm_eps; np.add = prio ? 2 : 0;
        if (l == 0) { np.emb = (const bf16_t*)Wp(c, "tok_embeddings.weight"); np.idx = sb.cur + b0; np.h_out = h; }
        if (l >= 0 && ctrl_at(l)) {
            np.add |= 1; np.ctrl = (const bf16_t*)c->ctrl[l / li].p + (size_t)b0 * n_tok * D; np.pos = cb.pos; np.T = T; np.n_tok = n_tok; np.cs = sb.cs; np.h_out = h;
        }
        np.pf_wgs = helpers_for(ra_norm, (b + 3) / 4);
        if (np.pf_wgs > 0) { wimg(pf0, np.pf_p0, np.pf_b0, cap0); if (!pf1.empty()) wimg(pf1, np.pf_p1, np.pf_b1); }
        car_launch_rmsnorm2(&np, b, st); ++nk;
    };
    auto normx_fields = [&](GemmDP& q, const std::string& wname) { q.nw = (const bf16_t*)Wp(c, wname); q.neps = g.norm_eps; q.nh_in = hc; q.ssq_in = fb.ssq; q.ssq_np = ssq_np; };
    auto norm_fields = [&](GemmDP& q, const std::string& wname, int l, bool first_of_layer) {
        q.nw = (const bf16_t*)Wp(c, wname); q.neps = g.norm_eps; q.nh_in = hc; q.pos = cb.pos;
        if (first_of_layer && l == 0) { q.nemb = (const bf16_t*)Wp(c, "tok_embeddings.weight"); q.nidx = sb.cur + b0; q.nh_out = h; }
        if (first_of_layer && ctrl_at(l)) {
            q.nadd = 1; q.nctrl = (const bf16_t*)c->ctrl[l / li].p + (size_t)b0 * n_tok * D; q.nT = T; q.n_tok = n_tok; q.ncs = sb.cs;
            q.nh_out = l == 0 ? h : (hc == h ? halt : h);
        }
    };
    auto norm_for = [&](GemmDP& q, bool nx, const std::string& wname, int l, bool first_of_layer, const std::string& pf0, const std::string& pf1, size_t cap0 = (size_t)24 << 20) {
        if (nx) normx_fields(q, wname);
        else if (cp.fuse_norm) norm_fields(q, wname, l, first_of_layer);
        else norm_kernel(wname, first_of_layer ? l : -1, pf0, pf1, cap0);
    };
    for (int l = 0; l < g.n_layer; ++l) {
        const std::string L = "layers." + std::to_string(l) + ".";
        const size_t kvb = g.kv_cache_fp8 ? 1 : 2;
        bf16_t* kc = (bf16_t*)((char*)c->kv.p + ((size_t)(2 * l) * kv_layer + kv_off) * kvb); bf16_t* vc = (bf16_t*)((char*)c->kv.p + ((size_t)(2 * l + 1) * kv_layer + kv_off) * kvb);
        const bool special = l == 0 || ctrl_at(l);
        const bool nx1 = cp.normx && !special && ssq_np > 0;
        {
            GemmDP q = z; q.qout = fb.q; q.kc = kc; q.vc = vc; q.rope = c->rope; q.pos = cb.pos; q.H = Hn; q.SA = SA; q.dim = D; q.kv8 = g.kv_cache_fp8 ? 1 : 0;
            norm_for(q, nx1, L + "attention_norm.weight", l, true, L + "attention.wqkv.weight", "");
            gemm(L + "attention.wqkv.weight", fb.xn, 3 * D, D, EPI_QKV, q);
            if (!nx1 && cp.fuse_norm && q.nh_out) hc = q.nh_out;
            if (l == 0 && phase_ev) { (void)hipEventRecord(phase_ev, st); (void)hipStreamWaitEvent(phase_dst, phase_ev, 0); }
        }
        {
            Attn2P ap; memset(&ap, 0, sizeof(ap));
            ap.q = fb.q; ap.kc = kc; ap.vc = vc; ap.pos = cb.pos; ap.mask = sb.maskb ? sb.maskb + (size_t)b0 * T : nullptr; ap.jmin = sb.jmin ? sb.jmin + b0 : nullptr;
            ap.out = fb.att; ap.part = fb.attn_part; ap.H = Hn; ap.SA = SA; ap.T = T; ap.dim = D; ap.nsplit = nsplit; ap.out_packed = 1; ap.kv8 = g.kv_cache_fp8 ? 1 : 0;
            if (cp.attn_pgrid > 0 && nsplit == 1) { ap.n_seq = b; ap.pgrid = cp.attn_pgrid; }
            if (cp.attn_variant == 162) {
                ap.pf_wgs = helpers_for(ra_lin, b * Hn);
                if (ap.pf_wgs > 0) { wimg(L + "attention.wo.weight", ap.pf_p0, ap.pf_b0); wimg(L + "feed_forward.w13.weight", ap.pf_p1, ap.pf_b1); }
            }
            car_launch_dec_attn2_var(&ap, b, cp.attn_variant, cp.attn_lds_pad, st); nk += nsplit > 1 ? 2 : 1;
        }
        { GemmDP q = z; q.h = hc; if (cp.normx) q.ssq_out = fb.ssq;
          if (cp.runahead == RA_SMALL) { q.pf_wgs = 1; wimg(L + "feed_forward.w2.weight", q.pf_p0, q.pf_b0); }
          else if (cp.runahead == RA_NX) { q.pf_wgs = 1; wimg(L + "feed_forward.w13.weight", q.pf_p0, q.pf_b0); wimg(L + "feed_forward.w2.weight", q.pf_p1, q.pf_b1); }
          ssq_np = gemm(L + "attention.wo.weight", fb.att, D, D, EPI_RESID, q); }
        { GemmDP q = z; q.outp = fb.mid;
          norm_for(q, cp.normx && ssq_np > 0, L + "ffn_norm.weight", l, false, L + "feed_forward.w13.weight", L + "feed_forward.w2.weight");
          gemm(L + "feed_forward.w13.weight", fb.xn, 2 * Fh, D, EPI_SWIGLU, q); }
        {
            GemmDP q = z; q.h = hc; if (cp.normx && !ctrl_at(l + 1)) q.ssq_out = fb.ssq;
            if (ra_lin) {
                q.pf_wgs = 1; wimg(l + 1 < g.n_layer ? "layers." + std::to_string(l + 1) + ".attention.wqkv.weight" : std::string("output.weight"), q.pf_p0, q.pf_b0, (size_t)16 << 20);
                if (l + 1 < g.n_layer && cp.kv_runahead) {
                    q.pf_kc = (const char*)c->kv.p + ((size_t)(2 * (l + 1)) * kv_layer + kv_off) * kvb; q.pf_vc = (const char*)c->kv.p + ((size_t)(2 * (l + 1) + 1) * kv_layer + kv_off) * kvb;
                    q.pf_pos = cb.pos; q.pf_items = b * Hn; q.pf_SA = SA; q.pf_kvb = (int)kvb;
                }
            }
            ssq_np = gemm(L + "feed_forward.w2.weight", fb.mid, D, Fh, EPI_RESID, q);
        }
    }
    { GemmDP q = z; q.outf = fb.logits;
      norm_for(q, cp.normx && ssq_np > 0, "norm.weight", g.n_layer, false, "output.weight", "", (size_t)16 << 20);
      gemm("output.weight", fb.xn, V, D, EPI_LOGITS, q); }
    car_launch_advance(cb.pos, cb.step, st); ++nk;
    SampleP sp = cb.sp; sp.logits = fb.logits; sp.logits_ks = 0; sp.round_bf16 = 0;
    car_launch_sample_greedy(&sp, st); ++nk;
    c->n_dec_kernels = nk;
    if (bad_cfg) FAIL(c, "decode GEMM: tile configuration %d rejected for this model's dimensions (b=%d, dim=%d, ffn=%d, vocab=%d)", bad_cfg, b, D, Fh, V);
    return 0;
}

static int enqueue_decode_step(car_ctx* c, const StepBufs& sb, const DecodePlan& pl, int ci, hipStream_t st, hipEvent_t phase_ev, hipStream_t phase_dst) {
    const car_config& g = c->cfg; const int mode = c->mode; const size_t e = c->esz;
    const ChainPlan& cp = pl.ch[ci]; const ChainBind& cb = sb.ch[ci];
    const int D = g.dim, Hn = g.n_head, Fh = g.ffn_hidden, li = g.n_layer / 3, V = g.vocab_size, T = g.cls_token_num;
    const int b = cp.bg, b0 = cp.b0, nsplit = cp.nsplit, S_max = sb.SA, n_tok = sb.n_tok;
    const size_t kv_layer = (size_t)sb.b * Hn * S_max * 64, kv_off = (size_t)b0 * Hn * S_max * 64;
    int nk = 0, bad = 0;
    auto gemm = [&](const std::string& wname, const void* X, long ldx, int N, int K, int epi, GemmFP q) {
        q.W = (const float*)Wp(c, wname + "#pk32"); q.X = (const float*)X; q.ldx = ldx; q.M = b; q.N = N; q.K = K;
        int cfg = car_pick_gemm_f32_cfg2(b, N, K, epi, sb.b / (b > 0 ? b : 1));
        if (K % 128 == 0 && N % 64 == 0) {
            if (epi == FEPI_RESID) { if (pl.f32_resid_cfg != kNoOverride && b >= 64) cfg = pl.f32_resid_cfg; }
            else if (N < 4096 && pl.f32_qkv_tiled_from != kNoOverride) cfg = b >= pl.f32_qkv_tiled_from ? 1212 : (b > 16 ? 22 : 21);
        }
        const int J = cfg % 10, Mb = (b + 15) / 16;
        q.w_nt = (cfg < 1000 && (Mb + J - 1) / J == 1 ? 1 : 0) | (pl.lin_prio ? 2 : 0);
        if (!q.W || car_launch_dec_gemm_f32_cfg(&q, epi, cfg, st)) bad = cfg ? cfg : -1;
        ++nk;
    };
    GemmFP z; memset(&z, 0, sizeof(z));
    GemmFP zn = z; zn.normx = 1; zn.neps = g.norm_eps;
    float* h = (float*)sb.h + (size_t)b0 * D; float* att = (float*)sb.att + (size_t)b0 * D;
    float* mid = (float*)sb.mid + (size_t)b0 * Fh; float* logits = sb.logits + (size_t)b0 * V; float* part = sb.part + (size_t)b0 * Hn * nsplit * 66;
    float* qbuf = (float*)sb.qkv + (size_t)b0 * D;
    for (int l = 0; l < g.n_layer; ++l) {
        const std::string L = "layers." + std::to_string(l) + ".";
        float* kc = (float*)off(c->kv.p, (size_t)(2 * l) * kv_layer + kv_off, e); float* vc = (float*)off(c->kv.p, (size_t)(2 * l + 1) * kv_layer + kv_off, e);
        const bool ctrl_here = sb.use_ctrl && l % li == 0 && l / li < 3;
        if (l == 0 || ctrl_here) {
            NormP np; memset(&np, 0, sizeof(np));
            np.h_in = h; np.h_out = h; np.xn = nullptr; np.D = D; np.eps = g.norm_eps;
            if (l == 0) { np.emb = Wp(c, "tok_embeddings.weight"); np.idx = sb.cur + b0; }
            if (ctrl_here) { np.add_mode = 1; np.ctrl = off(c->ctrl[l / li].p, (size_t)b0 * n_tok * D, e); np.pos = cb.pos; np.T = T; np.n_tok = n_tok; np.cs = sb.cs; }
            car_launch_rmsnorm(mode, &np, b, st); ++nk;
        }
        { GemmFP q = zn; q.qout = qbuf; q.kc = kc; q.vc = vc; q.rope = c->rope; q.pos = cb.pos; q.H = Hn; q.S_max = S_max; q.dim = D;
          gemm(L + "attention.wqkv.weight", h, D, 3 * D, D, FEPI_QKV, q); }
        if (l == 0 && phase_ev) { (void)hipEventRecord(phase_ev, st); (void)hipStreamWaitEvent(phase_dst, phase_ev, 0); }
        {
            AttnFP ap; memset(&ap, 0, sizeof(ap));
            ap.q = qbuf; ap.kc = kc; ap.vc = vc; ap.pos = cb.pos; ap.mask = sb.maskb ? sb.maskb + (size_t)b0 * T : nullptr; ap.part = part; ap.out = att;
            ap.H = Hn; ap.S_max = S_max; ap.T = T; ap.dim = D; ap.nsplit_max = nsplit;
            car_launch_dec_attn_f32_ex(&ap, b, cp.attn_variant, st); nk += cp.attn_variant ? 1 : 2;
        }
        { GemmFP q = z; q.out = h; q.ldo = D; q.R = h; gemm(L + "attention.wo.weight", att, D, D, D, FEPI_RESID, q); }
        { GemmFP q = zn; q.out = mid; q.ldo = Fh; gemm(L + "feed_forward.w13.weight", h, D, 2 * Fh, D, FEPI_SWIGLU, q); }
        { GemmFP q = z; q.out = h; q.ldo = D; q.R = h; gemm(L + "feed_forward.w2.weight", mid, Fh, D, Fh, FEPI_RESID, q); }
    }
    { GemmFP q = zn; q.out = logits; q.ldo = V; gemm("output.weight", h, D, V, D, FEPI_PLAIN, q); }
    car_launch_advance(cb.pos, cb.step, st); ++nk;
    SampleP sp = cb.sp; sp.logits = logits; sp.step_ptr = cb.step; car_launch_sample_greedy(&sp, st); ++nk;
    c->n_dec_kernels = nk;
    if (bad) FAIL(c, "exact-mode decode GEMM: tile configuration %d rejected (b=%d, dim=%d, ffn=%d, vocab=%d: N %% 32 and K %% 16 must be 0)", bad, b, D, Fh, V);
    return 0;
}

static int generate_impl(car_ctx* c, const void* text_emb, int32_t text_dtype, const int64_t* labels, const int64_t* emb_mask, int32_t B, int32_t n_new,
                         int32_t use_control, const car_sampling* sp, int32_t* out_tokens, const int32_t* forced_tokens,
                         float* logits_out, void* stream_);

extern "C" int car_generate(car_ctx* c, const void* text_emb, int32_t text_dtype, const int64_t* emb_mask, int32_t B, int32_t n_new,
                            int32_t use_control, const car_sampling* sp, int32_t* out_tokens, const int32_t* forced_tokens,
                            float* logits_out, void* stream_) {
    if (!c) return -1;
    if (c->cfg.model_type != 0) FAIL(c, "car_generate: context was created for the c2i model; use car_generate_c2i");
    if (!text_emb) FAIL(c, "car_generate: bad arguments");
    if (text_dtype != CAR_DT_F32 && text_dtype != CAR_DT_BF16) FAIL(c, "car_generate: text dtype must be F32 or BF16");
    return generate_impl(c, text_emb, text_dtype, nullptr, emb_mask, B, n_new, use_control, sp, out_tokens, forced_tokens, logits_out, stream_);
}

extern "C" int car_generate_c2i(car_ctx* c, const int64_t* labels, int32_t B, int32_t n_new, int32_t use_control, const car_sampling* sp,
                                int32_t* out_tokens, const int32_t* forced_tokens, float* logits_out, void* stream_) {
    if (!c) return -1;
    if (c->cfg.model_type != 1) FAIL(c, "car_generate_c2i: context was created for the t2i model; use car_generate");
    if (!labels) FAIL(c, "car_generate_c2i: bad arguments");
    return generate_impl(c, nullptr, CAR_DT_F32, labels, nullptr, B, n_new, use_control, sp, out_tokens, forced_tokens, logits_out, stream_);
}

static int generate_impl(car_ctx* c, const void* text_emb, int32_t text_dtype, const int64_t* labels, const int64_t* emb_mask, int32_t B, int32_t n_new,
                         int32_t use_control, const car_sampling* sp, int32_t* out_tokens, const int32_t* forced_tokens,
                         float* logits_out, void* stream_) {
    if (check_sticky(c)) return -1;
#ifdef CAR_DEV_KNOBS
    struct KnobLatch { car_ctx* c; int at_entry; ~KnobLatch() { const int d = g_car_knob_hits - at_entry; if (d > c->knob_hits) c->knob_hits = d; } } knob_latch{c, g_car_knob_hits};
#endif
    if (!c->finalized) FAIL(c, "car_generate: call car_finalize_weights first");
    if (!c->has_gpt) FAIL(c, "car_generate: this context holds VQ weights only");
    if (!sp || !out_tokens || B <= 0 || n_new <= 0) FAIL(c, "car_generate: bad arguments");
    const car_config& g = c->cfg;
    const bool c2i = g.model_type == 1;
    if (sp->sample_logits && g.vocab_size > 32768) FAIL(c, "car_generate: stochastic sampling supports vocab_size <= 32768");
    if (g.vocab_size % 4) FAIL(c, "car_generate: vocab_size must be a multiple of 4");
    const int T = g.cls_token_num;
    if (n_new > g.block_size) FAIL(c, "car_generate: max_new_tokens %d exceeds block_size %d (rope table rows, gpt_t2i.py:454)", n_new, g.block_size);
    if (use_control && (c->ctrl_B != B || c->ctrl_ntok < n_new)) FAIL(c, "car_generate: control tokens cached for B=%d n=%d, requested B=%d n_new=%d", c->ctrl_B, c->ctrl_ntok, B, n_new);
    const bool use_cfg = sp->cfg_scale > 1.0f;
    const int b = use_cfg ? 2 * B : B;
    const float cs = (use_cfg && !c2i) ? sp->control_strength : 1.0f;
    const int S_max = (int)rup(T + n_new, 8);
    const int SA = c->mode == CAR_BF16 ? (int)rup(S_max, 32) : S_max;
    const int D = g.dim, Hn = g.n_head, Fh = g.ffn_hidden, V = g.vocab_size, n_tok = c->ctrl_ntok, li = g.n_layer / 3;
    const int mode = c->mode; const size_t e = c->esz;
    hipStream_t caller = (hipStream_t)stream_, st = c->stream;
    const int Tpad = (int)rup(T, 32);

    const bool fast = mode == CAR_BF16;
    { int skip = 0; const char* ev = CAR_KNOB("CAR_DEBUG_SKIP_STEPS"); if (ev) { skip = atoi(ev); if (skip < 0 || skip > n_new - 2) skip = 0; } c->dbg_skip = skip; }
    const int nsteps = n_new - 1 - c->dbg_skip;
    DecodePlan pl; plan_decode(pl, g, mode, c->n_cu, B, use_cfg, S_max, nsteps, c->dbg_skip, emb_mask != nullptr);
    const int NG = pl.NG, mult = pl.mult; const int* img0 = pl.img0;
    std::vector<int> row_img((size_t)b), row_unc((size_t)b);
    for (int gi = 0; gi < NG; ++gi) {
        const int ng = img0[gi + 1] - img0[gi], base = mult * img0[gi];
        for (int j = 0; j < ng; ++j) { row_img[(size_t)base + j] = img0[gi] + j; row_unc[(size_t)base + j] = 0;
                                       if (use_cfg) { row_img[(size_t)base + ng + j] = img0[gi] + j; row_unc[(size_t)base + ng + j] = 1; } }
    }

    const size_t kv_layer = (size_t)b * Hn * SA * 64;
    const size_t kv_cap_before = c->kv.cap;
    const size_t kv_e = (fast && g.kv_cache_fp8) ? 1 : e;
    NEED(c, c->kv, (size_t)g.n_layer * 2 * kv_layer * kv_e);
    const bool kv_fresh = c->kv.cap != kv_cap_before;
    const long rowsP = (long)b * T;
    NEED(c, c->ws[0], (size_t)b * T * g.caption_dim * e);
    NEED(c, c->ws[1], (size_t)rowsP * D * e);
    NEED(c, c->ws[2], (size_t)rowsP * D * e);
    NEED(c, c->ws[3], (size_t)rowsP * 3 * D * e);
    const bool pf_flash = use_flash(c, 64);
    if (!pf_flash) {
        NEED(c, c->ws[4], (size_t)b * Hn * T * T * 4);
        NEED(c, c->ws[5], (size_t)b * Hn * T * Tpad * e);
    }
    NEED(c, c->ws[6], (size_t)b * D * Tpad * e);
    NEED(c, c->ws[7], (size_t)rowsP * (mode == CAR_BF16 ? Fh : 3 * Fh) * e);
    NEED(c, c->ws[8], (size_t)rowsP * D * e);
    NEED(c, c->ws[9], (size_t)b * V * 4);
    const int nsplit = fast ? attn_splits(b * Hn) : pl.ch[0].nsplit;
    NEED(c, c->ws[10], (size_t)b * Hn * nsplit * 66 * 4);
    NEED(c, c->ws[11], (size_t)B * (use_control ? n_tok : 1) * D * e);
    NEED(c, c->scal, (size_t)(16 + 2 * b + 4) * 4 + 16 + sizeof(SampleDyn) + 16);
    NEED(c, c->rowimg, (size_t)b * 4);
    NEED(c, c->tok_out, (size_t)B * n_new * 4);
    NEED(c, c->maskb, (size_t)b * T);
    for (int k = 0; k < 3; ++k) if (use_control) NEED(c, c->ctrl[k], (size_t)b * n_tok * D * e);

    fence_in(c, caller);
    HIPCHK(c, hipEventRecord(c->ev_t0, st));
    if (kv_fresh) HIPCHK(c, hipMemsetAsync(c->kv.p, 0, c->kv.cap, st));
    c->h_rowimg.assign(row_img.begin(), row_img.end());
    HIPCHK(c, hipMemcpyAsync(c->rowimg.p, c->h_rowimg.data(), (size_t)b * 4, hipMemcpyHostToDevice, st));
    car_launch_build_mask(emb_mask, (const int*)c->rowimg.p, (unsigned char*)c->maskb.p, b, T, st);
    int* pos = (int*)c->scal.p; int* step = pos + 1; int* cur = pos + 16; int* jmin = cur + b; int* jmin_min = jmin + b;
    SampleDyn* dyn = (SampleDyn*)(((uintptr_t)(jmin_min + 4) + 15) & ~(uintptr_t)15);
    c->h_dyn.seed = sp->seed; c->h_dyn.temperature = sp->temperature; c->h_dyn.top_k = sp->top_k; c->h_dyn.top_p = sp->top_p;
    HIPCHK(c, hipMemcpyAsync(dyn, &c->h_dyn, sizeof(SampleDyn), hipMemcpyHostToDevice, st));
    if (emb_mask) car_launch_mask_first_valid((const unsigned char*)c->maskb.p, jmin, b, T, st);
    int Tv = T, t0 = 0;
    if (emb_mask && !c2i && T > 8 && T % 8 == 0 && (mode == CAR_BF16 || T <= 128) && !CAR_KNOB("CAR_NO_PREFILL_WINDOW")) {
        int hmin = 0;
        const bool hinted = sp->first_valid_hint > 0;
        if (hinted) {
            hmin = sp->first_valid_hint - 1;
        } else {
            car_launch_min_int(jmin, b, jmin_min, -1, nullptr, st);
            HIPCHK(c, hipMemcpyAsync(&hmin, jmin_min, 4, hipMemcpyDeviceToHost, st));
            HIPCHK(c, hipStreamSynchronize(st));
        }
        const int hm = hmin < 0 ? 0 : (hmin > T ? T : hmin);
        t0 = (hm / 16) * 16; if (t0 > T - 8) t0 = ((T - 8) / 16) * 16; if (t0 < 0) t0 = 0;
        Tv = T - t0;
        if (Tv % 8) { Tv = T; t0 = 0; }
        if (hinted && t0 > 0) {
            if (!c->host_flags) { HIPCHK(c, hipHostMalloc((void**)&c->host_flags, 64, hipHostMallocMapped)); memset(c->host_flags, 0, 64); }
            car_launch_min_int(jmin, b, jmin_min, t0, c->host_flags + 1, st);
        }
    }
    const unsigned char* pmask = (const unsigned char*)c->maskb.p;
    if (t0 > 0) {
        NEED(c, c->maskw, (size_t)b * Tv);
        HIPCHK(c, hipMemcpy2DAsync(c->maskw.p, (size_t)Tv, (const unsigned char*)c->maskb.p + t0, (size_t)T, (size_t)Tv, (size_t)b, hipMemcpyDeviceToDevice, st));
        pmask = (const unsigned char*)c->maskw.p;
    }
    const long rowsW = (long)b * Tv;
    const int Tpw = (int)rup(Tv, 32);
    for (int i = 0; i < 8; ++i) { c->h_init[2 * i] = T + c->dbg_skip; c->h_init[2 * i + 1] = c->dbg_skip; }
    car_launch_set_pos_step(pos, c->h_init[0], c->h_init[1], st);

    void *text = c->ws[0].p, *h = c->ws[1].p, *xn = c->ws[2].p, *qkv = c->ws[3].p, *P = c->ws[5].p, *vT = c->ws[6].p, *mid = c->ws[7].p, *att = c->ws[8].p;
    float* S = (float*)c->ws[4].p; float* logits = (float*)c->ws[9].p;
    if (c2i) {
        c->h_rowunc.assign(row_unc.begin(), row_unc.end());
        NEED(c, c->rowunc, (size_t)b * 4 + 16);
        if (!c->host_flags) { HIPCHK(c, hipHostMalloc((void**)&c->host_flags, 64, hipHostMallocMapped)); memset(c->host_flags, 0, 64); }
        HIPCHK(c, hipMemcpyAsync(c->rowunc.p, c->h_rowunc.data(), (size_t)b * 4, hipMemcpyHostToDevice, st));
        int* didx = cur;
        car_launch_label_index(labels, (const int*)c->rowimg.p, (const int*)c->rowunc.p, g.num_classes, didx, c->host_flags, b, st);
        car_launch_gather_rows(mode, Wp(c, "cls_embedding.embedding_table.weight"), didx, h, b, D, st);
    } else {
        const long per_src = (long)T * g.caption_dim, per = (long)Tv * g.caption_dim; const size_t ib = text_dtype == CAR_DT_BF16 ? 2 : 4;
        for (int gi = 0; gi < NG; ++gi)
            car_launch_build_text(mode, (const char*)text_emb + (size_t)img0[gi] * per_src * ib, text_dtype, Wp(c, "cls_embedding.uncond_embedding"),
                                  off(text, (size_t)mult * img0[gi] * per, e), img0[gi + 1] - img0[gi], per, per_src, (long)t0 * g.caption_dim, use_cfg, st);
        mlp_tanh(c, text, g.caption_dim, 0, 1, (int)rowsW, g.caption_dim, "cls_embedding.cap_proj.", xn, h, D, st);
    }
    if (use_control) {
        const int Mc = B * n_tok;
        void* ce = c->ws[11].p;
        DevBuf& scratch = c->ws[4];
        const size_t s_bytes = pf_flash ? 0 : (size_t)b * Hn * T * T * 4;
        NEED(c, scratch, (size_t)Mc * D * e > s_bytes ? (size_t)Mc * D * e : s_bytes);
        S = (float*)c->ws[4].p;
        mlp_tanh(c, c->ctrl_in.p, D, 0, 1, Mc, D, "condition_mlp.cap_proj.", scratch.p, ce, D, st);
        for (int k = 0; k < 3; ++k) for (int gi = 0; gi < NG; ++gi) {
            const int ng = img0[gi + 1] - img0[gi]; const size_t rows = (size_t)ng * n_tok, base = (size_t)mult * img0[gi] * n_tok;
            mlp_tanh(c, off(ce, (size_t)img0[gi] * n_tok * D, e), D, 0, 1, (int)rows, D, "condition_layers." + std::to_string(k) + ".", scratch.p,
                     off(c->ctrl[k].p, base * D, e), D, st);
            if (use_cfg) HIPCHK(c, hipMemsetAsync(off(c->ctrl[k].p, (base + rows) * D, e), 0, rows * D * e, st));
        }
    }
    for (int l = 0; l < g.n_layer; ++l) {
        const std::string L = "layers." + std::to_string(l) + ".";
        {
            NormP np; memset(&np, 0, sizeof(np));
            np.h_in = h; np.h_out = h; np.xn = xn; np.w = Wp(c, L + "attention_norm.weight"); np.D = D; np.eps = g.norm_eps;
            if (use_control && l % li == 0 && l / li < 3) { np.add_mode = 2; np.ctrl = c->ctrl[l / li].p; np.T = Tv; np.n_tok = n_tok; np.cs = cs; }
            car_launch_rmsnorm(mode, &np, rowsW, st);
        }
        { GemmP q = gp(xn, D, Wp(c, L + "attention.wqkv.weight"), D, qkv, 3 * D, (int)rowsW, 3 * D, D); car_launch_gemm(mode, AMODE_PLAIN, &q, st); }
        if (fast) car_launch_prefill_rope_kv2(qkv, off(c->kv.p, (size_t)(2 * l) * kv_layer, kv_e), off(c->kv.p, (size_t)(2 * l + 1) * kv_layer, kv_e), c->rope, b, Tv, Hn, D, SA, g.kv_cache_fp8 ? 1 : 0, t0, st);
        else car_launch_prefill_rope_kv(mode, qkv, off(c->kv.p, (size_t)(2 * l) * kv_layer, e), off(c->kv.p, (size_t)(2 * l + 1) * kv_layer, e), c->rope, b, Tv, Hn, D, S_max, t0, st);
        car_launch_transpose_pad(mode, off(qkv, (size_t)2 * D, e), 3 * D, (long)Tv * 3 * D, vT, b, Tv, Tpw, D, st);
        bool fused = false;
        if (pf_flash) {
            FlashP f; memset(&f, 0, sizeof(f));
            f.q = (const bf16_t*)qkv; f.k = (const bf16_t*)qkv + D; f.vt = (const bf16_t*)vT; f.o = (bf16_t*)att;
            f.q_sb = f.k_sb = (long)Tv * 3 * D; f.q_st = f.k_st = 3 * D; f.vt_sb = (long)D * Tpw; f.vt_ld = Tpw; f.o_sb = (long)Tv * D; f.o_st = D;
            f.Tq = f.Tk = Tv; f.H = Hn; f.scale = 0.125f; f.mode = 1; f.mask = pmask;
            fused = car_launch_flash64(&f, b, st) == 0;
        }
        if (!fused) {
            GemmP q = gp(qkv, 3 * D, off(qkv, (size_t)D, e), 3 * D, S, Tv, Tv, Tv, 64);
            q.alpha = 0.125f; q.out_f32 = 1; q.nb0 = b; q.nb1 = Hn;
            q.sA0 = (long)Tv * 3 * D; q.sA1 = 64; q.sW0 = (long)Tv * 3 * D; q.sW1 = 64; q.sC0 = (long)Hn * Tv * Tv; q.sC1 = (long)Tv * Tv;
            car_launch_gemm(mode, AMODE_PLAIN, &q, st);
            car_launch_softmax_at(mode, S, Tv, P, Tpw, (long)b * Hn * Tv, Tv, 1, pmask, Tv, Hn, t0, st);
        }
        if (!fused) {
            GemmP q = gp(P, Tpw, vT, Tpw, att, D, Tv, 64, Tpw);
            q.nb0 = b; q.nb1 = Hn;
            q.sA0 = (long)Hn * Tv * Tpw; q.sA1 = (long)Tv * Tpw; q.sW0 = (long)D * Tpw; q.sW1 = (long)64 * Tpw; q.sC0 = (long)Tv * D; q.sC1 = 64;
            car_launch_gemm(mode, AMODE_PLAIN, &q, st);
        }
        { GemmP q = gp(att, D, Wp(c, L + "attention.wo.weight"), D, h, D, (int)rowsW, D, D); q.R = h; q.ldr = D; car_launch_gemm(mode, AMODE_PLAIN, &q, st); }
        { NormP np; memset(&np, 0, sizeof(np)); np.h_in = h; np.xn = xn; np.w = Wp(c, L + "ffn_norm.weight"); np.D = D; np.eps = g.norm_eps; car_launch_rmsnorm(mode, &np, rowsW, st); }
        if (mode == CAR_BF16) {
            GemmP q = gp(xn, D, Wp(c, L + "feed_forward.w13.weight"), D, mid, Fh, (int)rowsW, 2 * Fh, D); q.swiglu = 1; car_launch_gemm(mode, AMODE_PLAIN, &q, st);
        } else {
            void* mid2 = off(mid, (size_t)rowsW * Fh, e);
            GemmP q = gp(xn, D, Wp(c, L + "feed_forward.w13.weight"), D, mid2, 2 * Fh, (int)rowsW, 2 * Fh, D); car_launch_gemm(mode, AMODE_PLAIN, &q, st);
            car_launch_swiglu(mode, mid2, mid, rowsW, Fh, st);
        }
        { GemmP q = gp(mid, Fh, Wp(c, L + "feed_forward.w2.weight"), Fh, h, D, (int)rowsW, D, Fh); q.R = h; q.ldr = D; car_launch_gemm(mode, AMODE_PLAIN, &q, st); }
    }
    { NormP np; memset(&np, 0, sizeof(np)); np.h_in = h; np.xn = xn; np.w = Wp(c, "norm.weight"); np.D = D; np.eps = g.norm_eps; car_launch_rmsnorm(mode, &np, rowsW, st); }
    { GemmP q = gp(off(xn, (size_t)(Tv - 1) * D, e), (long)Tv * D, Wp(c, "output.weight"), D, logits, V, b, V, D); q.out_f32 = 1; car_launch_gemm(mode, AMODE_PLAIN, &q, st); }
    SampleP spp; memset(&spp, 0, sizeof(spp));
    spp.logits = logits; spp.B = B; spp.V = V; spp.use_cfg = use_cfg; spp.cfg_scale = sp->cfg_scale; spp.cfg_interval = sp->cfg_interval;
    spp.step_ptr = step; spp.n_new = n_new; spp.out_tokens = (int*)c->tok_out.p; spp.cur_tok = cur; spp.forced = forced_tokens; spp.logits_out = logits_out;
    spp.stochastic = sp->sample_logits != 0; spp.temperature = sp->temperature; spp.top_k = sp->top_k; spp.top_p = sp->top_p; spp.seed = sp->seed; spp.row0 = 0;
    spp.dyn = dyn;
    auto group_sampler = [&](int gi) {
        SampleP q = spp; const int i0 = img0[gi], ng = img0[gi + 1] - i0; const size_t rb = (size_t)mult * i0;
        q.B = ng; q.row0 = i0; q.logits = logits + rb * V; q.out_tokens = (int*)c->tok_out.p + (size_t)i0 * n_new; q.cur_tok = cur + rb;
        q.forced = forced_tokens ? forced_tokens + (size_t)i0 * n_new : nullptr;
        q.logits_out = logits_out ? logits_out + (size_t)i0 * n_new * V : nullptr;
        return q;
    };
    for (int gi = 0; gi < NG; ++gi) { SampleP q = group_sampler(gi); car_launch_sample_greedy(&q, st); }
    HIPCHK(c, hipEventRecord(c->ev_t1, st));

    StepBufs sb; memset(&sb, 0, sizeof(sb));
    sb.h = h; sb.xn = xn; sb.qkv = qkv; sb.att = att; sb.mid = mid; sb.part = (float*)c->ws[10].p; sb.logits = logits; sb.cur = cur;
    sb.b = b; sb.SA = SA; sb.n_tok = n_tok; sb.use_ctrl = use_control != 0; sb.cs = cs;
    sb.maskb = emb_mask ? (const unsigned char*)c->maskb.p : nullptr; sb.jmin = emb_mask ? jmin : nullptr;
    c->stats.graph_used = 0;
    for (int gi = 0; gi < NG; ++gi) {
        ChainBind& cb = sb.ch[gi];
        cb.pos = pos + 2 * gi; cb.step = step + 2 * gi; cb.sp = group_sampler(gi); cb.sp.step_ptr = cb.step;
    }
    { ChainBind& cb = sb.ch[kEarlyChain]; cb.pos = pos; cb.step = step; cb.sp = spp; }
    if (fast) {
        auto carve = [&](uintptr_t base) -> size_t {
            size_t o = 0;
            auto take = [&](size_t bytes) { void* p = (void*)(base + o); o += bytes; return p; };
            for (int gi = 0; gi < NG; ++gi) {
                const size_t bg = (size_t)pl.ch[gi].bg, M16 = rup(bg, 16); FastBufs& f = sb.ch[gi].fb;
                f.xn = (bf16_t*)take(M16 * D * 2); f.att = (bf16_t*)take(M16 * D * 2); f.mid = (bf16_t*)take(M16 * Fh * 2); f.q = (bf16_t*)take(rup(bg * D * 2, 16));
                f.logits = (float*)take(bg * V * 4); f.attn_part = (float*)take(rup(bg * Hn * pl.ch[gi].nsplit * 66 * 4, 16)); f.ssq = (float*)take(rup(M16 * (size_t)(D / 16) * 4, 16));
            }
            return o;
        };
        NEED(c, c->dec_parts, carve(0));
        carve((uintptr_t)c->dec_parts.p);
    }
    bool capturing = false; int step_rc = 0;
    const auto step_one = fast ? enqueue_decode_step_fast : enqueue_decode_step;
    auto enqueue_steps = [&](int k, bool early) {
        const int c0 = early ? kEarlyChain : 0, n = early ? 1 : NG, phase = early ? 0 : pl.phase;
        if (n >= 2 && capturing) {
            if (!phase) {
                (void)hipEventRecord(c->ev_fork, st);
                for (int gi = 1; gi < n; ++gi) (void)hipStreamWaitEvent(c->streamx[gi - 1], c->ev_fork, 0);
            }
            for (int gi = 0; gi < n; ++gi) {
                hipStream_t sg = gi == 0 ? st : c->streamx[gi - 1];
                for (int s = 0; s < k; ++s) {
                    const bool hand = phase && s == 0 && gi + 1 < n;
                    step_rc |= step_one(c, sb, pl, c0 + gi, sg, hand ? c->ev_phase[gi] : nullptr, hand ? c->streamx[gi] : nullptr);
                }
                if (gi > 0) { (void)hipEventRecord(c->ev_joinx[gi - 1], sg); (void)hipStreamWaitEvent(st, c->ev_joinx[gi - 1], 0); }
            }
        } else {
            for (int s = 0; s < k; ++s)
                for (int gi = 0; gi < n; ++gi) step_rc |= step_one(c, sb, pl, c0 + gi, st, nullptr, nullptr);
        }
        c->n_dec_kernels *= n;
    };
    if (nsteps > 0) {
        struct GraphShapes {
            int b, B, S_max, n_new, n_tok, nsplit, use_control, has_mask, cfg_interval, sample_logits; float cs, cfg_scale; unsigned long long alloc_gen;
            const void *kv, *h, *xn, *att, *mid, *logits, *ctrl0, *maskb, *parts, *scal, *forced, *logits_out;
        } gs;
        memset(&gs, 0, sizeof(gs));
        gs.b = b; gs.B = B; gs.S_max = S_max; gs.n_new = n_new; gs.n_tok = n_tok; gs.nsplit = nsplit; gs.use_control = use_control; gs.has_mask = emb_mask ? 1 : 0;
        gs.cfg_interval = sp->cfg_interval; gs.sample_logits = sp->sample_logits; gs.cs = cs; gs.cfg_scale = sp->cfg_scale; gs.alloc_gen = g_alloc_gen;
        gs.kv = c->kv.p; gs.h = h; gs.xn = xn; gs.att = att; gs.mid = mid; gs.logits = logits; gs.ctrl0 = c->ctrl[0].p; gs.maskb = c->maskb.p;
        gs.parts = c->dec_parts.p ? c->dec_parts.p : c->ws[10].p; gs.scal = c->scal.p; gs.forced = forced_tokens; gs.logits_out = logits_out;
        std::string key((const char*)&pl, sizeof(pl)); key.append((const char*)&gs, sizeof(gs));
        auto get_exec = [&](hipGraphExec_t& ex, std::string& exkey, int k, bool early = false) -> bool {
            const std::string kk = key + "|k" + std::to_string(k) + (early ? "|early" : "");
            if (ex && exkey == kk) return true;
            if (ex) { (void)hipGraphExecDestroy(ex); ex = nullptr; exkey.clear(); }
            hipGraph_t graph = nullptr;
            if (hipStreamBeginCapture(st, hipStreamCaptureModeThreadLocal) != hipSuccess) { (void)hipGetLastError(); return false; }
            capturing = true; enqueue_steps(k, early); capturing = false;
            bool ok = hipStreamEndCapture(st, &graph) == hipSuccess && graph != nullptr;
            if (!ok) (void)hipGetLastError();
            if (ok && hipGraphInstantiate(&ex, graph, nullptr, nullptr, 0) != hipSuccess) { ok = false; ex = nullptr; (void)hipGetLastError(); }
            if (graph) (void)hipGraphDestroy(graph);
            if (ok) exkey = kk;
            return ok;
        };
        const int n_early = pl.n_early, gsteps = pl.gsteps, nmain = nsteps - n_early;
        const int nrep = nmain / gsteps, nrem = nmain % gsteps;
        bool graph_ok = !pl.no_graph;
        for (int i = 0; i < 8; ++i) { c->h_init2[2 * i] = c->h_init[0] + n_early; c->h_init2[2 * i + 1] = c->h_init[1] + n_early; }
        if (graph_ok && n_early > 0) graph_ok = get_exec(c->gexec1, c->gkey1, 1, true);
        if (graph_ok && nrep > 0) graph_ok = get_exec(c->gexec, c->gkey, gsteps);
        if (graph_ok && nrem > 0) graph_ok = get_exec(gsteps > 1 ? c->gexec1 : c->gexec, gsteps > 1 ? c->gkey1 : c->gkey, 1);
        if (graph_ok && !step_rc) {
            for (int i = 0; i < n_early; ++i) HIPCHK(c, hipGraphLaunch(c->gexec1, st));
            if (n_early > 0 && nmain > 0) car_launch_set_pos_step(pos, c->h_init2[0], c->h_init2[1], st);
            for (int i = 0; i < nrep; ++i) HIPCHK(c, hipGraphLaunch(c->gexec, st));
            for (int i = 0; i < nrem; ++i) HIPCHK(c, hipGraphLaunch(gsteps > 1 ? c->gexec1 : c->gexec, st));
            c->stats.graph_used = 1;
        } else if (!step_rc) {
            for (int i = 0; i < n_early; ++i) enqueue_steps(1, true);
            if (n_early > 0 && nmain > 0) car_launch_set_pos_step(pos, c->h_init2[0], c->h_init2[1], st);
            for (int i = 0; i < nmain; ++i) enqueue_steps(1, false);
        }
    }
    if (step_rc) { fence_out(c, caller); return -1; }
    HIPCHK(c, hipEventRecord(c->ev_t2, st));
    HIPCHK(c, hipMemcpyAsync(out_tokens, c->tok_out.p, (size_t)B * n_new * 4, hipMemcpyDeviceToDevice, st));
    fence_out(c, caller);
    HIPCHK(c, hipGetLastError());
    {
        c->stats.decode_steps = nsteps;
        c->stats.decode_kernels_per_step = c->n_dec_kernels;
        const double we = (mode == CAR_BF16 && g.decode_weight_fp8) ? 1.0 : (double)e;
        c->st_wbytes = ((double)g.n_layer * ((double)3 * D * D + (double)D * D + 3.0 * (double)Fh * D) + (double)V * D) * we
                       + ((double)g.n_layer * 2.0 * D + D) * (double)e
                       + ((mode == CAR_BF16 && g.decode_weight_fp8) ? 4.0 * ((double)g.n_layer * (5.0 * D + 2.0 * Fh) + V) : 0.0);
        c->st_b = b; c->st_T = T; c->st_nsteps = nsteps; c->st_has_mask = emb_mask ? 1 : 0; c->st_jmin = jmin;
    }
    return 0;
}
```

controlar_amd/csrc/engine_internal.h:

```cpp
#pragma once
#include "car_common.h"
#include "../../include/controlar_hip.h"

#include <algorithm>
#include <cmath>
#include <cstdio>
#include <cstdlib>
#include <cstring>
#include <map>
#include <string>
#include <unordered_map>
#include <vector>

#include "decode2_params.h"
#include "decode_f32_params.h"
#include "kernel_params.h"
extern "C" {
int car_launch_dec_gemm_cfg(const GemmDP* p, int epi, int cfg, hipStream_t st);
int car_launch_dec_gemm_cfg_ex(const GemmDP* p, int epi, int cfg, int staged_ok, hipStream_t st);
int car_pick_gemm_cfg(int M, int N, int K, int epi);
void car_launch_dec_attn2_var(const Attn2P* p, int b, int variant, int lds_pad, hipStream_t st);
void car_launch_mask_first_valid(const unsigned char* mask, int* jmin, int b, int T, hipStream_t st);
void car_launch_prefill_rope_kv2(void* qkv, void* kc, void* vc, const float* rope, int b, int Tn, int H, int dim, int SA, int kv8, int t0, hipStream_t st);
void car_launch_min_int(const int* v, int n, int* out, int need, int* flag, hipStream_t st);
void car_launch_rmsnorm2(const Norm2P* p, long rows, hipStream_t st);
void car_launch_build_mask(const int64_t* emb_mask, const int* row_img, unsigned char* out, int b, int T, hipStream_t st);
void car_launch_canny_grad_nms(const unsigned char* img, unsigned char* map, int B, int H, int W, int low, int high, hipStream_t st);
void car_launch_canny_hyst(unsigned char* map, int B, int H, int W, const int* prev, int* changed, hipStream_t st);
void car_launch_canny_finish(int mode, const unsigned char* map, unsigned char* edges, void* control, int B, long HW, hipStream_t st);
void car_launch_rows_to_bf16(const void* src, int dtype, void* dst, long N, long K, int ileave, hipStream_t st);
void car_launch_pack_frag_bf16(const void* src, void* dst, long N, long K, hipStream_t st);
void car_launch_row_amax_scale(const void* src, int dtype, float* scale, long N, long K, int ileave, hipStream_t st);
void car_launch_quant_pack_fp8(const void* src, int dtype, const float* scale, void* rowmajor, void* pk, long N, long K, int ileave, hipStream_t st);
void car_launch_t5_prep(const long long* ids, const long long* mask, int* ids32, unsigned char* mk, long n, int vocab, hipStream_t st);
void car_launch_t5_softmax(int mode, const float* S, long lds, void* P, long ldp, long rows, int ncols, const float* bias,
                           const unsigned char* mask, int Tq, int n_head, hipStream_t st);
void car_launch_t5_gated_act(int mode, const void* in, void* out, long rows, int hidden, hipStream_t st);
int car_launch_flash64(const FlashP* p, int B, hipStream_t st);
int car_launch_gemm(int mode, int amode, const GemmP* p, hipStream_t st);
int car_conv3_halo64_ok(int mode, const GemmP* p);
void car_launch_convert(int mode, const void* src, int src_dtype, void* dst, long n, hipStream_t st);
void car_launch_build_text(int mode, const void* cond, int src_dtype, const void* uncond, void* dst, int B, long per, long per_src, long src_off, int use_cfg, hipStream_t st);
void car_launch_layernorm(int mode, const void* x, const void* w, const void* b, void* y, long rows, int D, float eps, hipStream_t st);
void car_launch_rmsnorm(int mode, const NormP* p, long rows, hipStream_t st);
void car_launch_softmax(int mode, const float* S, long lds, void* P, long ldp, long rows, int ncols, int mask_mode,
                        const unsigned char* emb_mask, int Tq, int n_head, hipStream_t st);
void car_launch_softmax_at(int mode, const float* S, long lds, void* P, long ldp, long rows, int ncols, int mask_mode,
                           const unsigned char* emb_mask, int Tq, int n_head, int col0, hipStream_t st);
void car_launch_patchify(int mode, const void* img, int img_dtype, void* out, int B, int H, int W, int gh, int gw, int p, int Kpad,
                         int bicubic, const int* iy, const int* ix, const float* wy, const float* wx, hipStream_t st);
void car_launch_vit_assemble(int mode, const void* tok, const void* cls, const void* pos, void* h, int B, int n, int D, hipStream_t st);
void car_launch_groupnorm(int mode, const void* x, const void* gamma, const void* beta, void* y, float* part, float* stats,
                          int B, int HW, int C, int G, float eps, int swish, hipStream_t st);
void car_launch_groupnorm_ex(int mode, const void* x, const void* gamma, const void* beta, void* y, float* part, float* stats, int B, int HW, int C, int G, float eps, int swish, int have_part, hipStream_t st);
void car_launch_vq_lookup(int mode, const int* tok, const float* cb, const float* wpq, const float* bpq, void* z, long npix, int cd, int zc, int ncode, hipStream_t st);
void car_launch_conv_in3(int mode, const float* img, const void* w, const void* b, void* out, int B, int H, int W, int Co, hipStream_t st);
void car_launch_vq_argmin(int mode, const void* z, const float* cb, int* tok, long npix, int cd, int ncode, hipStream_t st);
void car_launch_conv_out(int mode, const void* x, const void* w, const float* bias, float* out, int B, int H, int W, int C, hipStream_t st);
void car_launch_swiglu(int mode, const void* in, void* out, long rows, int hidden, hipStream_t st);
void car_launch_sample_greedy(const SampleP* p, hipStream_t st);
void car_launch_advance(int* pos, int* step, hipStream_t st);
void car_launch_set_pos_step(int* dst, int pos, int step, hipStream_t st);
void car_launch_transpose_pad(int mode, const void* src, long ld, long sb, void* dst, int B, int Tn, int Tpad, int C, hipStream_t st);
void car_launch_gather_rows(int mode, const void* table, const int* idx, void* out, long rows, int D, hipStream_t st);
void car_launch_label_index(const int64_t* labels, const int* row_img, const int* row_unc, int num_classes, int* idx, int* err_flag, int b, hipStream_t st);
void car_launch_prefill_rope_kv(int mode, void* qkv, void* kc, void* vc, const float* rope, int b, int Tn, int H, int dim, int S_max, int t0, hipStream_t st);
void car_launch_pack_frag_f32(const void* src, void* dst, long N, long K, const void* colscale, hipStream_t st);
int car_launch_dec_gemm_f32_cfg(const GemmFP* p, int epi, int cfg, hipStream_t st);
int car_pick_gemm_f32_cfg(int M, int N, int K, int epi);
int car_pick_gemm_f32_cfg2(int M, int N, int K, int epi, int chains);
void car_launch_dec_attn_f32(const AttnFP* p, int b, hipStream_t st);
void car_launch_dec_attn_f32_ex(const AttnFP* p, int b, int fused, hipStream_t st);
}


extern unsigned long long g_alloc_gen;
struct DevBuf {
    void* p = nullptr; size_t cap = 0;
    bool ensure(size_t bytes) {
        if (bytes <= cap) return true;
        if (p) (void)hipFree(p);
        p = nullptr; cap = 0;
        ++g_alloc_gen;
        size_t want = bytes + (bytes >> 3) + 256;
        if (hipMalloc(&p, want) != hipSuccess) { p = nullptr; return false; }
        cap = want; return true;
    }
    void release() { if (p) (void)hipFree(p); p = nullptr; cap = 0; }
};

struct Wt { void* p = nullptr; std::vector<int64_t> shape; int64_t numel = 0; size_t bytes = 0; };

struct car_ctx {
    car_config cfg; int mode = 0; size_t esz = 4;
    std::string err;
    hipStream_t streamx[7] = {}; hipEvent_t ev_fork = nullptr, ev_joinx[7] = {}, ev_phase[7] = {};
    hipStream_t stream = nullptr; hipEvent_t ev_in = nullptr, ev_out = nullptr, ev_t0 = nullptr, ev_t1 = nullptr, ev_t2 = nullptr;
    std::unordered_map<std::string, Wt> w;
    std::unordered_map<std::string, std::vector<float>> host_keep;
    std::unordered_map<std::string, int> w13_seen;
    bool finalized = false, has_gpt = false;
    std::map<std::pair<int, int>, void*> pos_cache;
    struct ResizeTab { int* iy; int* ix; float* wy; float* wx; };
    std::map<std::pair<int, int>, ResizeTab> resize_cache;
    float* rope = nullptr; int rope_rows = 0;
    DevBuf ctrl_in;
    int ctrl_B = 0, ctrl_ntok = 0;
    DevBuf ctrl[3];
    DevBuf kv;
    DevBuf ws[12];
    DevBuf dec_parts;
    DevBuf scal;
    DevBuf tok_out;
    DevBuf maskb;
    DevBuf maskw;
    std::vector<int> h_rowimg;
    int h_init[16] = {};
    int h_init2[16] = {};
    SampleDyn h_dyn = {};
    int dbg_skip = 0;
    int knob_hits = 0;
    int n_cu = 256;
    DevBuf rowimg;
    DevBuf rowunc; std::vector<int> h_rowunc;
    int* host_flags = nullptr;
    DevBuf canny_map;
    DevBuf lineart_ws;
    car_t5_config t5 = {}; bool has_t5 = false;
    DevBuf t5_in;
    DevBuf t5_bias; int t5_bias_T = 0;
    int st_b = 0, st_T = 0, st_nsteps = 0, st_has_mask = 0; double st_wbytes = 0; const int* st_jmin = nullptr;
    hipGraphExec_t gexec = nullptr; std::string gkey;
    hipGraphExec_t gexec1 = nullptr; std::string gkey1;
    car_stats stats;
    int n_dec_kernels = 0;
};

#define FAIL(ctx, ...) do { char _b[512]; snprintf(_b, sizeof(_b), __VA_ARGS__); (ctx)->err = _b; return -1; } while (0)
#define HIPCHK(ctx, x) do { hipError_t _e = (x); if (_e != hipSuccess) FAIL(ctx, "%s failed: %s (%s:%d)", #x, hipGetErrorString(_e), __FILE__, __LINE__); } while (0)
static inline int check_sticky(car_ctx* c) {
    if (!c->host_flags) return 0;
    volatile int* f = c->host_flags;
    if (f[1]) { f[1] = 0; FAIL(c, "car_generate: an earlier call passed a first_valid_hint beyond the first valid prompt position of its batch: valid prompt rows were left out of the prefill, its tokens are invalid"); }
    if (f[0]) { f[0] = 0; FAIL(c, "car_generate_c2i: an earlier call on this context received a class label outside [0, %d] (clamped to the null class on the device): its tokens are invalid", c->cfg.num_classes); }
    return 0;
}
#define NEED(ctx, buf, bytes) do { if (!(buf).ensure(bytes)) FAIL(ctx, "out of device memory allocating %zu bytes (%s:%d)", (size_t)(bytes), __FILE__, __LINE__); } while (0)

static inline size_t rup(size_t x, size_t a) { return (x + a - 1) / a * a; }


static inline bool ends_with(const std::string& s, const char* suf) { size_t n = strlen(suf); return s.size() >= n && s.compare(s.size() - n, n, suf) == 0; }
static inline bool starts_with(const std::string& s, const char* pre) { return s.compare(0, strlen(pre), pre) == 0; }

static inline const void* Wp(car_ctx* c, const std::string& name) {
    auto it = c->w.find(name);
    return it == c->w.end() ? nullptr : it->second.p;
}

struct VqItem { int kind; std::string name; int cin, cout; };
static inline std::vector<VqItem> vq_layout(const car_config& g, int* last_c) {
    std::vector<VqItem> v;
    const int nres = g.vq_n_mult;
    int block_in = g.vq_ch * g.vq_ch_mult[nres - 1];
    v.push_back({0, "decoder.mid.0", block_in, block_in}); v.push_back({1, "decoder.mid.1", block_in, block_in}); v.push_back({0, "decoder.mid.2", block_in, block_in});
    for (int idx = 0; idx < nres; ++idx) {
        const int i_level = nres - 1 - idx, block_out = g.vq_ch * g.vq_ch_mult[i_level];
        for (int j = 0; j < g.vq_num_res_blocks + 1; ++j) {
            v.push_back({0, "decoder.conv_blocks." + std::to_string(idx) + ".res." + std::to_string(j), block_in, block_out});
            block_in = block_out;
            if (i_level == nres - 1) v.push_back({1, "decoder.conv_blocks." + std::to_string(idx) + ".attn." + std::to_string(j), block_in, block_in});
        }
        if (i_level != 0) v.push_back({2, "decoder.conv_blocks." + std::to_string(idx) + ".upsample", block_in, block_in});
    }
    *last_c = block_in;
    return v;
}

static inline std::vector<VqItem> vq_enc_layout(const car_config& g, int* last_c) {
    std::vector<VqItem> v;
    const int nres = g.vq_n_mult;
    int block_in = g.vq_ch;
    for (int i = 0; i < nres; ++i) {
        block_in = g.vq_ch * (i == 0 ? 1 : g.vq_ch_mult[i - 1]);
        const int block_out = g.vq_ch * g.vq_ch_mult[i];
        for (int j = 0; j < g.vq_num_res_blocks; ++j) {
            v.push_back({0, "encoder.conv_blocks." + std::to_string(i) + ".res." + std::to_string(j), block_in, block_out});
            block_in = block_out;
            if (i == nres - 1) v.push_back({1, "encoder.conv_blocks." + std::to_string(i) + ".attn." + std::to_string(j), block_in, block_in});
        }
        if (i != nres - 1) v.push_back({3, "encoder.conv_blocks." + std::to_string(i) + ".downsample", block_in, block_in});
    }
    v.push_back({0, "encoder.mid.0", block_in, block_in}); v.push_back({1, "encoder.mid.1", block_in, block_in}); v.push_back({0, "encoder.mid.2", block_in, block_in});
    *last_c = block_in;
    return v;
}

static inline GemmP gp(const void* A, long lda, const void* W, long ldw, void* C, long ldc, int M, int N, int K) {
    GemmP p; memset(&p, 0, sizeof(p));
    p.A = A; p.W = W; p.C = C; p.lda = lda; p.ldw = ldw; p.ldc = ldc; p.M = M; p.N = N; p.K = K;
    p.alpha = 1.f; p.nb0 = 1; p.nb1 = 1;
    return p;
}
static inline char* off(void* p, size_t elems, size_t esz) { return (char*)p + elems * esz; }
static inline const char* off(const void* p, size_t elems, size_t esz) { return (const char*)p + elems * esz; }

static inline bool use_flash(const car_ctx* c, int head_dim) {
    static const bool off_env = CAR_KNOB("CAR_NO_FLASH") != nullptr;
    return c->mode == CAR_BF16 && head_dim == 64 && !off_env;
}

static inline void mlp_tanh(car_ctx* c, const void* x, long lda, long sA, int nb, int M, int K, const std::string& pfx, void* mid, void* y, int dim, hipStream_t st) {
    GemmP p = gp(x, lda, Wp(c, pfx + "fc1.weight"), K, mid, dim, M, dim, K);
    p.act = ACT_GELU_TANH; p.nb0 = nb; p.sA0 = sA; p.sC0 = (long)M * dim;
    car_launch_gemm(c->mode, AMODE_PLAIN, &p, st);
    GemmP q = gp(mid, dim, Wp(c, pfx + "fc2.weight"), dim, y, dim, M * nb, dim, dim);
    car_launch_gemm(c->mode, AMODE_PLAIN, &q, st);
}

static inline void fence_in(car_ctx* c, hipStream_t caller) { (void)hipEventRecord(c->ev_in, caller); (void)hipStreamWaitEvent(c->stream, c->ev_in, 0); }
static inline void fence_out(car_ctx* c, hipStream_t caller) { (void)hipEventRecord(c->ev_out, c->stream); (void)hipStreamWaitEvent(caller, c->ev_out, 0); }

int get_resize(car_ctx* c, int H, int W, int nh, int nw, car_ctx::ResizeTab* out);
int get_pos_embed(car_ctx* c, int gh, int gw, void** out);
```

Measured before the change: 43.80.

## Add packed on-the-fly RMSNorm GEMM variant for large decode batches

Adds a NORM==4 decode GEMM variant. The residual-add producer also writes a fragment-packed copy of h, and the next GEMM reads that copy through the normal X path, folding rmsnorm from partial sums of squares on the fly. It is enabled for batch sizes above the existing normx limit, which previously fell back to a separate rmsnorm launch. This removes one kernel and an activation round trip per norm. The cost is an extra packed write in the epilogue and a block-wide sync to share rstd values.

Result: slower. 40.67 (-7.1%).

```diff
diff --git a/controlar_amd/csrc/decode2.hip b/controlar_amd/csrc/decode2.hip
--- a/controlar_amd/csrc/decode2.hip
+++ b/controlar_amd/csrc/decode2.hip
@@ -85,10 +85,13 @@
 __global__ __launch_bounds__(WAVES * 64) void dec_gemm_kernel(GemmDP p) {
     extern __shared__ __attribute__((aligned(16))) float red_all[];
     static_assert((NORM != 1 && NORM != 3) || J == 1, "the prologue-norm and staged-norm variants serve one m-block");
+    static_assert(NORM != 4 || (F8 == 0 && J <= WAVES), "the packed on-the-fly norm: bf16 weights, one folding wave per m-block");
     const int xs_ld = p.K + 8;
     bf16_t* xs = (bf16_t*)red_all;
     float* red = NORM == 1 ? red_all + (16 * xs_ld) / 2 : (NORM == 3 ? red_all + ((size_t)WAVES * p.stg) / 4 : red_all);
     constexpr int XPU = F8 ? 2 : 1;
+    constexpr bool NX = NORM == 2 || NORM == 4;
+    constexpr int NRW = NX ? XPU : 1;
     if (J == 1 && WAVES >= 8) car_kernarg_prefetch<(sizeof(GemmDP) + 63 + 48) / 64>();
     const int tid = threadIdx.x, lane = tid & 63, wave = tid >> 6;
     if (p.pf_wgs > 0 && (int)blockIdx.x >= (int)gridDim.x - p.pf_wgs) {
@@ -118,23 +121,23 @@
         for (int j = 0; j < J; ++j) acc[i][j] = (f32x4){0.f, 0.f, 0.f, 0.f};
     const u32x4 zw = (u32x4){0u, 0u, 0u, 0u};
     constexpr int DEPTH = WAVES == 16 ? 8 : ((28 / (I + J * XPU)) < 2 ? 2 : ((28 / (I + J * XPU)) > 6 ? 6 : (28 / (I + J * XPU))));
-    u32x4 wr[DEPTH][I], xr[DEPTH][J * XPU], nr[DEPTH][NORM == 2 ? XPU : 1];
+    u32x4 wr[DEPTH][I], xr[DEPTH][J * XPU], nr[DEPTH][NRW];
     const bf16_t* hrow[J]; bool hok[J]; float rstd[J];
 #pragma unroll
-    for (int j = 0; j < J; ++j) { const int m = (mb0 + j) * 16 + (lane & 15); hok[j] = NORM == 2 && m < p.M; hrow[j] = NORM == 2 ? p.nh_in + (long)(hok[j] ? m : 0) * p.K + (lane >> 4) * 8 : nullptr; rstd[j] = 0.f; }
-    auto loadW = [&](u32x4 (&w)[I], u32x4 (&nwf)[NORM == 2 ? XPU : 1], int ku) {
+    for (int j = 0; j < J; ++j) { const int m = (mb0 + j) * 16 + (lane & 15); hok[j] = NX && m < p.M; hrow[j] = NORM == 2 ? p.nh_in + (long)(hok[j] ? m : 0) * p.K + (lane >> 4) * 8 : nullptr; rstd[j] = 0.f; }
+    auto loadW = [&](u32x4 (&w)[I], u32x4 (&nwf)[NRW], int ku) {
 #pragma unroll
         for (int i = 0; i < I; ++i) {
             const u32x4* a = wp + ((long)i * nku + ku) * 64;
             w[i] = (p.w_nt & 1) ? __builtin_nontemporal_load(a) : *a;
         }
-        if (NORM == 2) {
+        if (NX) {
 #pragma unroll
             for (int u = 0; u < XPU; ++u) nwf[u] = *(const u32x4*)(p.nw + (ku * XPU + u) * 32 + (lane >> 4) * 8);
         }
     };
     auto loadX = [&](u32x4 (&x)[J * XPU], int ku) {
-        if (NORM == 0) {
+        if (NORM == 0 || NORM == 4) {
 #pragma unroll
             for (int j = 0; j < J; ++j)
 #pragma unroll
@@ -146,7 +149,7 @@
                 for (int u = 0; u < XPU; ++u) { x[j * XPU + u] = zw; if (hok[j]) x[j * XPU + u] = *(const u32x4*)(hrow[j] + (ku * XPU + u) * 32); }
         }
     };
-    auto load = [&](u32x4 (&w)[I], u32x4 (&x)[J * XPU], u32x4 (&nwf)[NORM == 2 ? XPU : 1], int ku) { loadW(w, nwf, ku); loadX(x, ku); };
+    auto load = [&](u32x4 (&w)[I], u32x4 (&x)[J * XPU], u32x4 (&nwf)[NRW], int ku) { loadW(w, nwf, ku); loadX(x, ku); };
     const bf16_t* xl = xs + (lane & 15) * xs_ld + (lane >> 4) * 8;
     const int s_nkbw = NORM == 3 ? (ku_hi - ku_lo) * XPU : 0;
     const int s_xr = NORM == 3 ? (p.M * ((nku + WAVES - 1) / WAVES) * XPU * 4 + 63) >> 6 : 0;
@@ -154,7 +157,7 @@
     const char* stg_x = (const char*)red_all + (size_t)wave * (NORM == 3 ? p.stg : 0);
     const char* stg_w = stg_x + (size_t)s_xr * 1024;
     const char* stg_s = stg_w + 1024;
-    auto compute = [&](const u32x4 (&w)[I], u32x4 (&x)[J * XPU], const u32x4 (&nwf)[NORM == 2 ? XPU : 1], int ku) {
+    auto compute = [&](const u32x4 (&w)[I], u32x4 (&x)[J * XPU], const u32x4 (&nwf)[NRW], int ku) {
         if (NORM == 1) {
 #pragma unroll
             for (int u = 0; u < XPU; ++u) x[u] = *(const u32x4*)(xl + (ku * XPU + u) * 32);
@@ -171,7 +174,7 @@
                     x[u][e] = pack_bf16x2(__uint_as_float(t << 16) * __uint_as_float(wv << 16), __uint_as_float(t & 0xffff0000u) * __uint_as_float(wv & 0xffff0000u));
                 }
             }
-        } else if (NORM == 2) {
+        } else if (NX) {
 #pragma unroll
             for (int j = 0; j < J; ++j)
 #pragma unroll
@@ -282,6 +285,15 @@
 #pragma unroll
         for (int j = 0; j < J; ++j) { if (J <= 2) ssq_issue(sv[j], j); else { ssq_issue(sv[0], j); ssq_finish(sv[0], j); } }
     }
+    float4 pv[NORM == 4 ? 8 : 1];
+    const int m4 = (mb0 + wave) * 16 + (lane & 15);
+    const bool ok4 = NORM == 4 && wave < J && m4 < p.M;
+    if (NORM == 4 && wave < J) {
+        const int np4 = p.ssq_np >> 2, q4n = lane >> 4;
+        const float4* sp = (const float4*)(p.ssq_in + (long)m4 * p.ssq_np);
+#pragma unroll
+        for (int t = 0; t < 8; ++t) { pv[t] = make_float4(0.f, 0.f, 0.f, 0.f); if (ok4 && q4n + 4 * t < np4) { const u32x4 r = *(const u32x4*)(sp + q4n + 4 * t); pv[t] = make_float4(__uint_as_float(r[0]), __uint_as_float(r[1]), __uint_as_float(r[2]), __uint_as_float(r[3])); } }
+    }
 #pragma unroll
     for (int d = 0; d < DEPTH; ++d) if (d < nkw) load(wr[d], xr[d], nr[d], ku_lo + d);
     rope_first();
@@ -302,6 +314,19 @@
     if (NORM == 2 && J <= 2) {
 #pragma unroll
         for (int j = 0; j < J; ++j) ssq_finish(sv[J <= 2 ? j : 0], j);
+    }
+    if (NORM == 4) {
+        float* rs4 = red_all + (size_t)WAVES * I * J * 64 * 4;
+        if (wave < J) {
+            float sum = 0.f;
+#pragma unroll
+            for (int t = 0; t < 8; ++t) { sum += pv[t].x; sum += pv[t].y; sum += pv[t].z; sum += pv[t].w; }
+            sum += __shfl_xor(sum, 16, 64); sum += __shfl_xor(sum, 32, 64);
+            if (lane < 16) rs4[wave * 16 + lane] = ok4 ? rsqrtf(sum / p.K + p.neps) : 0.f;
+        }
+        __syncthreads();
+#pragma unroll
+        for (int j = 0; j < J; ++j) rstd[j] = rs4[j * 16 + (lane & 15)];
     }
     if (NORM == 1) {
         const int D = p.K, ng = D >> 2;
@@ -427,6 +452,10 @@
                     o.x = pack_bf16x2(h0 + bf2f(f2bf(a[0])), h1 + bf2f(f2bf(a[1])));
                     o.y = pack_bf16x2(h2 + bf2f(f2bf(a[2])), h3 + bf2f(f2bf(a[3])));
                     *(uint2*)hp = o;
+                    if (p.xp_out) {
+                        const long off = ((((long)(m >> 4) * (p.N >> 5) + (n0 >> 5)) * 64 + ((n0 & 31) >> 3) * 16 + (m & 15)) << 3) + (n0 & 7);
+                        *(uint2*)(p.xp_out + off) = o;
+                    }
                     if (p.ssq_out) {
                         const float s0 = __uint_as_float(o.x << 16), s1 = __uint_as_float(o.x & 0xffff0000u), s2 = __uint_as_float(o.y << 16), s3 = __uint_as_float(o.y & 0xffff0000u);
                         ssq_acc += s0 * s0; ssq_acc += s1 * s1; ssq_acc += s2 * s2; ssq_acc += s3 * s3;
@@ -488,7 +517,7 @@
         const int nku = p.K / (F8 ? 64 : 32), xr = (p.M * ((nku + WAVES - 1) / WAVES) * (F8 ? 2 : 1) * 4 + 63) / 64, sr = (p.M * (p.ssq_np / 4) + 63) / 64;
         p.stg = (xr + 1 + sr) * 1024;
     }
-    const size_t sh = (size_t)WAVES * I * J * 64 * 16 + (NORM == 1 ? (size_t)16 * (p.K + 8) * 2 : 0) + (NORM == 3 ? (size_t)WAVES * p.stg : 0);
+    const size_t sh = (size_t)WAVES * I * J * 64 * 16 + (NORM == 4 ? (size_t)64 * J : 0) + (NORM == 1 ? (size_t)16 * (p.K + 8) * 2 : 0) + (NORM == 3 ? (size_t)WAVES * p.stg : 0);
     static size_t attr[4] = {0, 0, 0, 0};
 #define LG(E)                                                                                                                   \
     do {                                                                                                                        \
@@ -503,13 +532,24 @@
 #undef LG
 }
 
+extern "C" int car_dec_gemm_packed_norm_ok(int cfg) { return cfg == 440 || cfg == 441 || cfg == 241 || cfg == 221 || cfg == 211 || cfg == 210 || cfg == 110; }
 extern "C" int car_launch_dec_gemm_cfg_ex(const GemmDP* p, int epi, int cfg, int staged_ok, hipStream_t st) {
     if (epi == EPI_SWIGLU && cfg < 200) return -1;
     if (p->N % (16 * (cfg / 100)) || p->K % 32) return -1;
     if (p->wscale && p->K % 64) return -1;
     const int f8 = p->wscale ? (p->f8_mfma ? 2 : 1) : 0;
     if (p->ssq_in) {
-        if (!p->nw || !p->nh_in || epi == EPI_RESID || p->ssq_np <= 0 || (p->ssq_np & 3) || p->ssq_np > 128) return -1;
+        if (!p->nw || (!p->nh_in && !p->norm_packed) || epi == EPI_RESID || p->ssq_np <= 0 || (p->ssq_np & 3) || p->ssq_np > 128) return -1;
+        if (p->norm_packed) {
+            if (f8 || !p->X || !car_dec_gemm_packed_norm_ok(cfg)) return -1;
+            switch (cfg) {
+#define CASE4(I, J, W) case I * 100 + J * 10 + (W == 8): launch_gemm_ij<I, J, W, 0, 4>(*p, epi, st); break;
+                CASE4(4, 4, 4) CASE4(4, 4, 8) CASE4(2, 4, 8) CASE4(2, 2, 8) CASE4(2, 1, 8) CASE4(2, 1, 4) CASE4(1, 1, 4)
+#undef CASE4
+                default: return -1;
+            }
+            return 0;
+        }
         {
             const int nku = p->K / (f8 ? 64 : 32), nkw_max = (nku + 7) / 8;
             if (p->M <= 16 && (cfg / 10) % 10 == 1 && cfg % 10 == 1 && nku >= 8 && nkw_max * (f8 ? 2 : 1) <= 16 && staged_ok) {
diff --git a/controlar_amd/csrc/decode2_params.h b/controlar_amd/csrc/decode2_params.h
--- a/controlar_amd/csrc/decode2_params.h
+++ b/controlar_amd/csrc/decode2_params.h
@@ -32,6 +32,7 @@
     const float* ssq_in; int ssq_np;
     int stg;
     float* ssq_out; int ssq_ld;
+    bf16_t* xp_out; int norm_packed;
     CAR_PF_FIELDS
     CAR_STAMP_FIELDS
 };
diff --git a/controlar_amd/csrc/engine_generate.hip b/controlar_amd/csrc/engine_generate.hip
--- a/controlar_amd/csrc/engine_generate.hip
+++ b/controlar_amd/csrc/engine_generate.hip
@@ -5,6 +5,7 @@
     int b0, bg, nsplit;
     int attn_variant, attn_lds_pad, attn_pgrid;
     int fuse_norm, normx, normx_max, normx_j4, staged_normx;
+    int normp;
     int runahead, kv_runahead;
 };
 struct DecodePlan {
@@ -24,7 +25,7 @@
     auto num = [](const char* v, int dflt) { return v ? atoi(v) : dflt; };
     const char *k_chains = CAR_KNOB("CAR_CHAINS"), *k_one_max = CAR_KNOB("CAR_ONE_LAUNCH_MAX"), *k_variant = CAR_KNOB("CAR_ATTN_VARIANT"), *k_phase = CAR_KNOB("CAR_PHASE_OFFSET"), *k_form = CAR_KNOB("CAR_ATTN_F32_FORM");
     const bool single_chain = CAR_KNOB("CAR_SINGLE_CHAIN"), no_early = CAR_KNOB("CAR_NO_EARLY_CHAIN"), split_small = CAR_KNOB("CAR_ATTN_SPLIT_SMALL"), old_small = CAR_KNOB("CAR_ATTN_OLD_SMALL");
-    const bool no_runahead = CAR_KNOB("CAR_NO_RUNAHEAD"), no_small_fuse = CAR_KNOB("CAR_NO_SMALL_FUSE"), no_normx = CAR_KNOB("CAR_NO_NORMX"), kv_runahead = CAR_KNOB("CAR_KV_RUNAHEAD"), no_staged = CAR_KNOB("CAR_NO_STAGED_NORMX");
+    const bool no_runahead = CAR_KNOB("CAR_NO_RUNAHEAD"), no_small_fuse = CAR_KNOB("CAR_NO_SMALL_FUSE"), no_normx = CAR_KNOB("CAR_NO_NORMX"), kv_runahead = CAR_KNOB("CAR_KV_RUNAHEAD"), no_staged = CAR_KNOB("CAR_NO_STAGED_NORMX"), no_normp = CAR_KNOB("CAR_NO_PACKED_NORMX");
     const int k_nsplit = num(CAR_KNOB("CAR_ATTN_NSPLIT"), 0), k_persist = num(CAR_KNOB("CAR_ATTN_PERSIST"), 0), lds_pad = num(CAR_KNOB("CAR_ATTN_LDS_PAD"), 0);
     const int normx_max = num(CAR_KNOB("CAR_NORMX_MAX"), 48), normx_j4 = num(CAR_KNOB("CAR_NORMX_J4"), 0) != 0, k_gsteps = num(CAR_KNOB("CAR_GRAPH_STEPS"), 1);
     pl.mode = mode; pl.mult = mult; pl.lin_prio = num(CAR_KNOB("CAR_LINEAR_PRIO"), 0) != 0;
@@ -56,6 +57,12 @@
         cp.fuse_norm = bg <= 8 && D <= 2048 && !no_small_fuse;
         cp.normx_max = normx_max; cp.normx_j4 = normx_j4; cp.staged_normx = !no_staged;
         cp.normx = bg <= normx_max && D % 128 == 0 && D <= 2048 && !no_normx;
+        {
+            const int ep[3] = {EPI_QKV, EPI_SWIGLU, EPI_LOGITS}, nn[3] = {3 * D, 2 * Fh, V};
+            bool tiles = true;
+            for (int i = 0; i < 3; ++i) tiles = tiles && car_dec_gemm_packed_norm_ok(car_pick_gemm_cfg(bg, nn[i], D, ep[i]));
+            cp.normp = NG >= 2 && bg > normx_max && bg > 48 && D % 128 == 0 && D <= 2048 && !g.decode_weight_fp8 && tiles && !no_normx && !no_normp;
+        }
         if (n_cu >= 128 && !no_runahead) cp.runahead = bg <= 16 ? RA_SMALL : (bg != b ? RA_NONE : (bg <= normx_max ? RA_NX : RA_MID));
         cp.kv_runahead = kv_runahead && cp.attn_variant == 162 && ((bg * Hn) & 7) == 0;
     }
@@ -102,7 +109,7 @@
         p.W = (const bf16_t*)Wp(c, wname + (f8 ? "#pk8" : "#pk")); p.X = X; p.M = b; p.N = N; p.K = K;
         p.wscale = f8 ? (const float*)Wp(c, wname + "#sc") : nullptr; p.f8_mfma = g.decode_weight_fp8 == 2;
         int cfg = car_pick_gemm_cfg(b, N, K, epi);
-        if (p.ssq_in && b > 48 && b <= 64 && cp.normx_j4) cfg = ((epi == EPI_SWIGLU || N >= 6144) ? 200 : 100) + 40 + 1;
+        if (p.ssq_in && !p.norm_packed && b > 48 && b <= 64 && cp.normx_j4) cfg = ((epi == EPI_SWIGLU || N >= 6144) ? 200 : 100) + 40 + 1;
         const int I = cfg / 100, J = (cfg / 10) % 10, Mb = (b + 15) / 16;
         p.w_nt = ((Mb + J - 1) / J == 1 ? 1 : 0) | (prio ? 2 : 0);
         if (p.pf_wgs > 0) p.pf_wgs = std::min(helpers_for(ra_lin, (N / (16 * I)) * ((Mb + J - 1) / J)), 160);
@@ -126,7 +133,8 @@
         if (np.pf_wgs > 0) { wimg(pf0, np.pf_p0, np.pf_b0, cap0); if (!pf1.empty()) wimg(pf1, np.pf_p1, np.pf_b1); }
         car_launch_rmsnorm2(&np, b, st); ++nk;
     };
-    auto normx_fields = [&](GemmDP& q, const std::string& wname) { q.nw = (const bf16_t*)Wp(c, wname); q.neps = g.norm_eps; q.nh_in = hc; q.ssq_in = fb.ssq; q.ssq_np = ssq_np; };
+    auto normx_fields = [&](GemmDP& q, const std::string& wname) { q.nw = (const bf16_t*)Wp(c, wname); q.neps = g.norm_eps; q.nh_in = hc; q.ssq_in = fb.ssq; q.ssq_np = ssq_np; q.norm_packed = cp.normp; };
+    const bool nxa = cp.normx || cp.normp;
     auto norm_fields = [&](GemmDP& q, const std::string& wname, int l, bool first_of_layer) {
         q.nw = (const bf16_t*)Wp(c, wname); q.neps = g.norm_eps; q.nh_in = hc; q.pos = cb.pos;
         if (first_of_layer && l == 0) { q.nemb = (const bf16_t*)Wp(c, "tok_embeddings.weight"); q.nidx = sb.cur + b0; q.nh_out = h; }
@@ -145,7 +153,7 @@
         const size_t kvb = g.kv_cache_fp8 ? 1 : 2;
         bf16_t* kc = (bf16_t*)((char*)c->kv.p + ((size_t)(2 * l) * kv_layer + kv_off) * kvb); bf16_t* vc = (bf16_t*)((char*)c->kv.p + ((size_t)(2 * l + 1) * kv_layer + kv_off) * kvb);
         const bool special = l == 0 || ctrl_at(l);
-        const bool nx1 = cp.normx && !special && ssq_np > 0;
+        const bool nx1 = nxa && !special && ssq_np > 0;
         {
             GemmDP q = z; q.qout = fb.q; q.kc = kc; q.vc = vc; q.rope = c->rope; q.pos = cb.pos; q.H = Hn; q.SA = SA; q.dim = D; q.kv8 = g.kv_cache_fp8 ? 1 : 0;
             norm_for(q, nx1, L + "attention_norm.weight", l, true, L + "attention.wqkv.weight", "");
@@ -164,15 +172,15 @@
             }
             car_launch_dec_attn2_var(&ap, b, cp.attn_variant, cp.attn_lds_pad, st); nk += nsplit > 1 ? 2 : 1;
         }
-        { GemmDP q = z; q.h = hc; if (cp.normx) q.ssq_out = fb.ssq;
+        { GemmDP q = z; q.h = hc; if (nxa) q.ssq_out = fb.ssq; if (cp.normp) q.xp_out = fb.xn;
           if (cp.runahead == RA_SMALL) { q.pf_wgs = 1; wimg(L + "feed_forward.w2.weight", q.pf_p0, q.pf_b0); }
           else if (cp.runahead == RA_NX) { q.pf_wgs = 1; wimg(L + "feed_forward.w13.weight", q.pf_p0, q.pf_b0); wimg(L + "feed_forward.w2.weight", q.pf_p1, q.pf_b1); }
           ssq_np = gemm(L + "attention.wo.weight", fb.att, D, D, EPI_RESID, q); }
         { GemmDP q = z; q.outp = fb.mid;
-          norm_for(q, cp.normx && ssq_np > 0, L + "ffn_norm.weight", l, false, L + "feed_forward.w13.weight", L + "feed_forward.w2.weight");
+          norm_for(q, nxa && ssq_np > 0, L + "ffn_norm.weight", l, false, L + "feed_forward.w13.weight", L + "feed_forward.w2.weight");
           gemm(L + "feed_forward.w13.weight", fb.xn, 2 * Fh, D, EPI_SWIGLU, q); }
         {
-            GemmDP q = z; q.h = hc; if (cp.normx && !ctrl_at(l + 1)) q.ssq_out = fb.ssq;
+            GemmDP q = z; q.h = hc; if (nxa && !ctrl_at(l + 1)) { q.ssq_out = fb.ssq; if (cp.normp) q.xp_out = fb.xn; }
             if (ra_lin) {
                 q.pf_wgs = 1; wimg(l + 1 < g.n_layer ? "layers." + std::to_string(l + 1) + ".attention.wqkv.weight" : std::string("output.weight"), q.pf_p0, q.pf_b0, (size_t)16 << 20);
                 if (l + 1 < g.n_layer && cp.kv_runahead) {
@@ -184,7 +192,7 @@
         }
     }
     { GemmDP q = z; q.outf = fb.logits;
-      norm_for(q, cp.normx && ssq_np > 0, "norm.weight", g.n_layer, false, "output.weight", "", (size_t)16 << 20);
+      norm_for(q, nxa && ssq_np > 0, "norm.weight", g.n_layer, false, "output.weight", "", (size_t)16 << 20);
       gemm("output.weight", fb.xn, V, D, EPI_LOGITS, q); }
     car_launch_advance(cb.pos, cb.step, st); ++nk;
     SampleP sp = cb.sp; sp.logits = fb.logits; sp.logits_ks = 0; sp.round_bf16 = 0;
diff --git a/controlar_amd/csrc/engine_internal.h b/controlar_amd/csrc/engine_internal.h
--- a/controlar_amd/csrc/engine_internal.h
+++ b/controlar_amd/csrc/engine_internal.h
@@ -19,6 +19,7 @@
 int car_launch_dec_gemm_cfg(const GemmDP* p, int epi, int cfg, hipStream_t st);
 int car_launch_dec_gemm_cfg_ex(const GemmDP* p, int epi, int cfg, int staged_ok, hipStream_t st);
 int car_pick_gemm_cfg(int M, int N, int K, int epi);
+int car_dec_gemm_packed_norm_ok(int cfg);
 void car_launch_dec_attn2_var(const Attn2P* p, int b, int variant, int lds_pad, hipStream_t st);
 void car_launch_mask_first_valid(const unsigned char* mask, int* jmin, int b, int T, hipStream_t st);
 void car_launch_prefill_rope_kv2(void* qkv, void* kc, void* vc, const float* rope, int b, int Tn, int H, int dim, int SA, int kv8, int t0, hipStream_t st);
diff --git a/experiments/normx_check.hip b/experiments/normx_check.hip
--- /dev/null
+++ b/experiments/normx_check.hip
@@ -0,0 +1,173 @@
+#include "../controlar_amd/csrc/decode2.hip"
+
+#include <cstdio>
+#include <cstdlib>
+#include <cstring>
+#include <cmath>
+#include <thread>
+#include <vector>
+#define CK(x) do { hipError_t e_ = (x); if (e_ != hipSuccess) { printf("HIP error %s at %s:%d\n", hipGetErrorString(e_), __FILE__, __LINE__); exit(2); } } while (0)
+
+static unsigned rs = 4242u;
+static float urand() { rs = rs * 1664525u + 1013904223u; return ((rs >> 8) & 0xffffff) / 16777216.0f; }
+static float rb(float v) { return bf2f(f2bf(v)); }
+static int g_fail = 0;
+
+static std::vector<bf16_t> pack_rows(const std::vector<float>& a, int R, int K, bf16_t pad) {
+    const int Rb = (R + 15) / 16, nkb = K / 32;
+    std::vector<bf16_t> o((size_t)Rb * 16 * K, pad);
+    for (int r = 0; r < R; ++r) for (int k = 0; k < K; ++k)
+        o[((((size_t)(r / 16) * nkb + k / 32) * 64 + ((k % 32) / 8) * 16 + r % 16) << 3) + k % 8] = f2bf(a[(size_t)r * K + k]);
+    return o;
+}
+template <typename T> static T* dalloc(size_t n) { T* p; CK(hipMalloc(&p, n * sizeof(T))); return p; }
+template <typename T> static void h2d(T* d, const std::vector<T>& h) { CK(hipMemcpy(d, h.data(), h.size() * sizeof(T), hipMemcpyHostToDevice)); }
+template <typename T> static std::vector<T> d2h(const T* d, size_t n) { std::vector<T> h(n); CK(hipMemcpy(h.data(), d, n * sizeof(T), hipMemcpyDeviceToHost)); return h; }
+
+static void report(const char* what, size_t bad, size_t n, double worst, bool bits) {
+    const bool ok = bad == 0;
+    if (!ok) ++g_fail;
+    if (bits) printf("%s: %zu of %zu %s\n", what, bad, n, ok ? "differ, ok" : "BITS DIFFER");
+    else printf("%s: worst |d| / tol %.3f, %zu of %zu beyond %s\n", what, worst, bad, n, ok ? "ok" : "FAIL");
+}
+
+static void check(int M, int K, int N) {
+    const int D = K, Kp = 64, Mb = (M + 15) / 16, M16 = Mb * 16, pos = 37, SA = 64, H = D / 64;
+    const float eps = 1e-5f;
+    char nm[200];
+    std::vector<float> Xp((size_t)M * Kp), Wp((size_t)D * Kp), h0((size_t)M * D), nw(D), W((size_t)N * K);
+    for (auto& v : Xp) v = rb(urand() * 2.f - 1.f);
+    for (auto& v : Wp) v = rb((urand() - 0.5f) * 0.5f);
+    for (auto& v : h0) v = rb((urand() - 0.5f) * 4.f);
+    for (auto& v : nw) v = rb(0.5f + urand());
+    for (auto& v : W) v = rb((urand() - 0.5f) * 0.2f);
+    std::vector<bf16_t> h0b(h0.size()), nwb(D);
+    for (size_t i = 0; i < h0.size(); ++i) h0b[i] = f2bf(h0[i]);
+    for (int i = 0; i < D; ++i) nwb[i] = f2bf(nw[i]);
+    const auto xpp = pack_rows(Xp, M, Kp, f2bf(0.f)), wpp = pack_rows(Wp, D, Kp, f2bf(0.f)), wpk = pack_rows(W, N, K, f2bf(0.f));
+    bf16_t *dXp = dalloc<bf16_t>(xpp.size()), *dWp = dalloc<bf16_t>(wpp.size()), *dW = dalloc<bf16_t>(wpk.size()), *dh = dalloc<bf16_t>(h0b.size()), *dxp = dalloc<bf16_t>((size_t)M16 * D), *dnw = dalloc<bf16_t>(D);
+    float* dssq = dalloc<float>((size_t)M16 * (D / 16));
+    h2d(dXp, xpp); h2d(dWp, wpp); h2d(dW, wpk); h2d(dh, h0b); h2d(dnw, nwb);
+    CK(hipMemset(dxp, 0xff, (size_t)M16 * D * 2)); CK(hipMemset(dssq, 0xff, (size_t)M16 * (D / 16) * 4));
+    const int pcfg = car_pick_gemm_cfg(M, D, Kp, EPI_RESID), pI = pcfg / 100, np = D / (16 * (pI >= 2 ? 2 : 1));
+    {
+        GemmDP p; memset(&p, 0, sizeof(p));
+        p.W = dWp; p.X = dXp; p.M = M; p.N = D; p.K = Kp; p.h = dh; p.ssq_out = dssq; p.ssq_ld = np; p.xp_out = dxp;
+        if (car_launch_dec_gemm_cfg(&p, EPI_RESID, pcfg, 0)) { printf("producer cfg %d rejected FAIL\n", pcfg); ++g_fail; return; }
+        CK(hipDeviceSynchronize()); CK(hipGetLastError());
+    }
+    const auto hb = d2h(dh, h0b.size()); const auto xpb = d2h(dxp, (size_t)M16 * D);
+    std::vector<float> hf(hb.size()); for (size_t i = 0; i < hb.size(); ++i) hf[i] = bf2f(hb[i]);
+    {
+        const auto want = pack_rows(hf, M, D, (bf16_t)0xffff);
+        size_t bad = 0; for (size_t i = 0; i < want.size(); ++i) if (memcmp(&want[i], &xpb[i], 2)) ++bad;
+        snprintf(nm, sizeof(nm), "M=%d D=%d producer cfg %d (np %d): packed copy vs host re-pack of h, pad rows untouched", M, D, pcfg, np); report(nm, bad, want.size(), 0, true);
+        size_t badh = 0; double worst = 0;
+        for (int m = 0; m < M; ++m) for (int n = 0; n < D; ++n) {
+            double s = 0; for (int k = 0; k < Kp; ++k) s += (double)Xp[(size_t)m * Kp + k] * Wp[(size_t)n * Kp + k];
+            const double w = (double)h0[(size_t)m * D + n] + rb((float)s), tol = fabs(w) / 256 + fabs(s) / 128 + 1e-3, d = fabs(hf[(size_t)m * D + n] - w);
+            worst = fmax(worst, d / tol); if (!(d <= tol)) ++badh;
+        }
+        snprintf(nm, sizeof(nm), "M=%d D=%d producer: h vs fp64 residual add", M, D); report(nm, badh, (size_t)M * D, worst, false);
+    }
+    std::vector<double> x((size_t)M * K), acc((size_t)M * N);
+    for (int m = 0; m < M; ++m) {
+        double ss = 0; for (int k = 0; k < K; ++k) ss += (double)hf[(size_t)m * K + k] * hf[(size_t)m * K + k];
+        const float rstd = (float)(1.0 / sqrt(ss / K + eps));
+        for (int k = 0; k < K; ++k) x[(size_t)m * K + k] = rb(rb(hf[(size_t)m * K + k] * rstd) * nw[k]);
+    }
+    {
+        std::vector<double> Wd(W.begin(), W.end());
+        std::vector<std::thread> th; const int NT = 8;
+        for (int t = 0; t < NT; ++t) th.emplace_back([&, t]() {
+            for (int m = t; m < M; m += NT) for (int n = 0; n < N; ++n) {
+                const double *a = &x[(size_t)m * K], *b = &Wd[(size_t)n * K]; double s0 = 0, s1 = 0, s2 = 0, s3 = 0;
+                for (int k = 0; k < K; k += 4) { s0 += a[k] * b[k]; s1 += a[k + 1] * b[k + 1]; s2 += a[k + 2] * b[k + 2]; s3 += a[k + 3] * b[k + 3]; }
+                acc[(size_t)m * N + n] = (s0 + s1) + (s2 + s3);
+            }
+        });
+        for (auto& t : th) t.join();
+    }
+    std::vector<float> rope((size_t)(pos + 1) * 64);
+    for (int q = 0; q <= pos; ++q) for (int i = 0; i < 32; ++i) { const float a = 0.01f * q * (i + 1); rope[((size_t)q * 32 + i) * 2] = cosf(a); rope[((size_t)q * 32 + i) * 2 + 1] = sinf(a); }
+    float* dR = dalloc<float>(rope.size()); h2d(dR, rope);
+    int* dPos = dalloc<int>(1); CK(hipMemcpy(dPos, &pos, 4, hipMemcpyHostToDevice));
+    const bool qkv_shape = N == 3 * D;
+    for (int epi : {EPI_LOGITS, EPI_SWIGLU, EPI_QKV}) {
+        if (epi == EPI_QKV && !qkv_shape) continue;
+        const int No = epi == EPI_SWIGLU ? N / 2 : N;
+        std::vector<double> want((size_t)M * No), tol((size_t)M * No);
+        for (int m = 0; m < M; ++m) for (int n = 0; n < No; ++n) {
+            const size_t o = (size_t)m * No + n; const double* am = &acc[(size_t)m * N];
+            if (epi == EPI_LOGITS) { want[o] = am[n]; tol[o] = fabs(am[n]) / 256 + 1e-3; }
+            else if (epi == EPI_SWIGLU) {
+                const double a = am[(2 * (n / 16)) * 16 + n % 16], c = am[(2 * (n / 16) + 1) * 16 + n % 16];
+                const double ar = rb((float)a), cr = rb((float)c), sg = 1.0 / (1.0 + exp(-ar)), si = rb((float)(ar * sg)), dsi = fabs(sg * (1.0 + ar * (1.0 - sg)));
+                want[o] = rb((float)(si * cr));
+                tol[o] = fabs(want[o]) / 256 + (dsi * fabs(ar) / 128 + fabs(si) / 128) * fabs(cr) + fabs(si) * fabs(cr) / 128 + 1e-3;
+            } else {
+                const int sec = n / D, d = n % D;
+                if (sec == 2) { want[o] = am[n]; tol[o] = fabs(am[n]) / 256 + 1e-3; }
+                else {
+                    const int d0 = d & ~1; const double x0 = rb((float)am[sec * D + d0]), x1 = rb((float)am[sec * D + d0 + 1]);
+                    const double cs = rope[((size_t)pos * 32 + ((d0 & 63) >> 1)) * 2], sn = rope[((size_t)pos * 32 + ((d0 & 63) >> 1)) * 2 + 1];
+                    const double r = (d & 1) ? x1 * cs + x0 * sn : x0 * cs - x1 * sn, sc = sec == 0 ? 0.125 : 1.0;
+                    want[o] = r * sc; tol[o] = (fabs(r) / 256 + (fabs(x0) + fabs(x1)) / 128 + 1e-3) * sc;
+                }
+            }
+        }
+        const size_t osz = epi == EPI_LOGITS ? (size_t)M * N * 2  : (epi == EPI_SWIGLU ? (size_t)M16 * No : 0);
+        const size_t csz = (size_t)M * H * SA * 64;
+        bf16_t* dO[2] = {nullptr, nullptr}; bf16_t *dK[2] = {nullptr, nullptr}, *dV[2] = {nullptr, nullptr}, *dQ[2] = {nullptr, nullptr};
+        for (int f = 0; f < 2; ++f) { if (osz) dO[f] = dalloc<bf16_t>(osz); if (epi == EPI_QKV) { dK[f] = dalloc<bf16_t>(csz); dV[f] = dalloc<bf16_t>(csz); dQ[f] = dalloc<bf16_t>((size_t)M * D); } }
+        for (int cfg : {440, 441, 241, 221, 211, 210, 110}) {
+            const int I = cfg / 100;
+            if (N % (16 * I) || (epi == EPI_SWIGLU && I < 2)) continue;
+            std::vector<bf16_t> out[2], ok_[2], ov[2], oq[2];
+            bool rejected = false;
+            for (int f = 0; f < 2; ++f) {
+                GemmDP p; memset(&p, 0, sizeof(p));
+                p.W = dW; p.M = M; p.N = N; p.K = K; p.nw = dnw; p.neps = eps; p.ssq_in = dssq; p.ssq_np = np;
+                if (f == 0) { p.X = dxp; p.norm_packed = 1; } else p.nh_in = dh;
+                if (epi == EPI_LOGITS) p.outf = (float*)dO[f]; else if (epi == EPI_SWIGLU) p.outp = dO[f];
+                else { p.qout = dQ[f]; p.kc = dK[f]; p.vc = dV[f]; p.rope = dR; p.pos = dPos; p.H = H; p.SA = SA; p.dim = D; }
+                if (osz) CK(hipMemset(dO[f], 0, osz * 2));
+                if (epi == EPI_QKV) { CK(hipMemset(dK[f], 0, csz * 2)); CK(hipMemset(dV[f], 0, csz * 2)); CK(hipMemset(dQ[f], 0, (size_t)M * D * 2)); }
+                if (car_launch_dec_gemm_cfg(&p, epi, cfg, 0)) { printf("cfg %d NORM %d rejected FAIL\n", cfg, f ? 2 : 4); ++g_fail; rejected = true; break; }
+                CK(hipDeviceSynchronize()); CK(hipGetLastError());
+                if (osz) out[f] = d2h(dO[f], osz);
+                if (epi == EPI_QKV) { ok_[f] = d2h(dK[f], csz); ov[f] = d2h(dV[f], csz); oq[f] = d2h(dQ[f], (size_t)M * D); }
+            }
+            if (rejected) continue;
+            size_t bad = 0, tot = 0;
+            auto cmp = [&](const std::vector<bf16_t>& a, const std::vector<bf16_t>& b) { tot += a.size(); for (size_t i = 0; i < a.size(); ++i) if (memcmp(&a[i], &b[i], 2)) ++bad; };
+            cmp(out[0], out[1]); cmp(ok_[0], ok_[1]); cmp(ov[0], ov[1]); cmp(oq[0], oq[1]);
+            const char* en = epi == EPI_LOGITS ? "LOGITS" : (epi == EPI_SWIGLU ? "SWIGLU" : "QKV");
+            snprintf(nm, sizeof(nm), "M=%d K=%d N=%d %s cfg %d: NORM 4 vs NORM 2 output bits", M, K, N, en, cfg); report(nm, bad, tot, 0, true);
+            size_t over = 0; double worst = 0;
+            for (int m = 0; m < M; ++m) for (int n = 0; n < No; ++n) {
+                float got;
+                if (epi == EPI_LOGITS) got = ((const float*)out[0].data())[(size_t)m * N + n];
+                else if (epi == EPI_SWIGLU) got = bf2f(out[0][((((size_t)(m / 16) * (No / 32) + n / 32) * 64 + ((n % 32) / 8) * 16 + m % 16) << 3) + n % 8]);
+                else {
+                    const int sec = n / D, hh = (n % D) / 64, d = n % 64; const size_t sb = ((size_t)m * H + hh) * SA * 64;
+                    if (sec == 0) got = bf2f(oq[0][(size_t)m * D + n]);
+                    else if (sec == 1) got = bf2f(ok_[0][sb + ((size_t)(pos / 16) * 2 + d / 32) * 512 + (((d % 32) / 8) * 16 + pos % 16) * 8 + d % 8]);
+                    else { const int w = pos % 32, qv = w < 16 ? w / 4 : (w - 16) / 4, ev = w < 16 ? w % 4 : 4 + (w - 16) % 4;
+                           got = bf2f(ov[0][sb + ((size_t)(pos / 32) * 4 + d / 16) * 512 + (qv * 16 + d % 16) * 8 + ev]); }
+                }
+                const size_t o = (size_t)m * No + n; const double dd = fabs((double)got - want[o]);
+                worst = fmax(worst, dd / tol[o]); if (!(dd <= tol[o])) ++over;
+            }
+            snprintf(nm, sizeof(nm), "M=%d K=%d N=%d %s cfg %d: NORM 4 vs fp64 rmsnorm + GEMM + epilogue", M, K, N, en, cfg); report(nm, over, (size_t)M * No, worst, false);
+        }
+        for (int f = 0; f < 2; ++f) for (void* b : {(void*)dO[f], (void*)dK[f], (void*)dV[f], (void*)dQ[f]}) if (b) CK(hipFree(b));
+    }
+    for (void* b : {(void*)dXp, (void*)dWp, (void*)dW, (void*)dh, (void*)dxp, (void*)dnw, (void*)dssq, (void*)dR, (void*)dPos}) CK(hipFree(b));
+}
+
+int main() {
+    for (int M : {49, 64, 200}) { check(M, 256, 768); check(M, 1280, 3840); check(M, 1280, 7168); }
+    printf(g_fail ? "FAILED: %d checks\n" : "all checks passed\n", g_fail);
+    return g_fail ? 1 : 0;
+}
```
